# soniareilly/HPCClassMultigridProject

Hardware: NVIDIA B200
Metric: V-cycle ms at N=16384^2 (fine-grid V-cycle incl. convergence check) (lower is better)
Workload: dtype f64

## Files before the change

hpcclassmultigridproject_b200/csrc/solver.cu:

```cuda
#include <cmath>
#include <cstdlib>
#include <cstring>
#include <mutex>
#include <string>
#include <utility>
#include <vector>

#include "comm.cuh"
#include "ops_basic.cuh"
#include "stream_pass.cuh"

namespace mgb200 {

static thread_local std::string g_last_error;
void set_error(const std::string& msg) { g_last_error = msg; }
int fail(int code, const std::string& msg)
{
    g_last_error = msg;
    return code;
}
long& launch_counter()
{
    static thread_local long c = 0;
    return c;
}

Stencil make_stencil(double dt, double nu, double dx)
{
    volatile double r = 0.5 * dt / (dx * dx);
    volatile double four_r = 4.0 * r;
    volatile double four_r_nu = four_r * nu;
    Stencil s;
    s.r = r; s.nu = nu; s.h = dx;
    s.diag = 1.0 - four_r_nu;
    s.diag_rhs = 1.0 + four_r_nu;
    s.inv_diag = 1.0 / s.diag;
    s.hr = r * dx * 0.5;
    s.rnu = r * nu;
    return s;
}

struct Level {
    long n = 0;
    Layout L{0, 0};
    Stencil st{};
    size_t elems = 0;
    double* u[2] = {nullptr, nullptr};
    int cur = 0;
    double *rhs = nullptr, *v1 = nullptr, *v2 = nullptr;
    long own_lo = 0, own_hi = 0;
    long mem_lo = 0, mem_hi = 0;
    bool sharded = false;
    bool present = true;
    long rows_mem() const { return mem_hi - mem_lo + 1; }
};

constexpr long SLAB_HALO = 8;

struct Slab { long own_lo, own_hi, mem_lo, mem_hi; };
static Slab slab_of(long n, int P, int rank)
{
    Slab w;
    const long per = n / P;
    w.own_lo = rank * per;
    w.own_hi = (rank + 1) * per - 1 + (rank == P - 1 ? 1 : 0);
    w.mem_lo = w.own_lo - SLAB_HALO < 0 ? 0 : w.own_lo - SLAB_HALO;
    w.mem_hi = w.own_hi + SLAB_HALO > n ? n : w.own_hi + SLAB_HALO;
    return w;
}
static Slab child_slab_of(long n_fine, int P, int rank)
{
    const Slab f = slab_of(n_fine, P, rank);
    const long nc = n_fine / 2;
    Slab w;
    w.own_lo = (f.own_lo + 1) / 2;
    w.own_hi = f.own_hi / 2;
    w.mem_lo = w.own_lo - SLAB_HALO < 0 ? 0 : w.own_lo - SLAB_HALO;
    w.mem_hi = w.own_hi + SLAB_HALO > nc ? nc : w.own_hi + SLAB_HALO;
    return w;
}

struct LoopState {
    double res0, tol;
    int iter, max_cycle;
    double hist[52];
};

__global__ void k_loop_begin(cudaGraphConditionalHandle h, const double* norm2, LoopState* st, double tol, int max_cycle)
{
    const double r0 = sqrt(norm2[0]);
    st->res0 = r0; st->tol = tol; st->iter = 0; st->max_cycle = max_cycle; st->hist[0] = r0;
    cudaGraphSetConditional(h, (0 < max_cycle && r0 / r0 > tol) ? 1u : 0u);
}

__global__ void k_loop_check(cudaGraphConditionalHandle h, const double* norm2, LoopState* st)
{
    const double r = sqrt(norm2[0]);
    const int it = ++st->iter;
    st->hist[it] = r;
    cudaGraphSetConditional(h, (it < st->max_cycle && r / st->res0 > st->tol) ? 1u : 0u);
}

}

using namespace mgb200;

struct mgb200_solver {
    long N = 0;
    int maxlvl = 0;
    double nu = 0, dt = 0, dx = 0, tol = 0;
    mgb200_options opt{};
    int device = 0;
    std::vector<Level> lv;
    cudaStream_t stream = nullptr;
    double* d_partials = nullptr;
    long partials_cap = 0;
    double* d_norm2 = nullptr;
    double* h_norm2 = nullptr;
    int* d_coarse_iters = nullptr;
    double* d_coarse_lu = nullptr;
    double* d_flat[2] = {nullptr, nullptr};
    cudaGraphExec_t graph_exec = nullptr;
    long graph_kernels = 0;
    cudaGraphExec_t loop_exec = nullptr;
    bool loop_failed = false;
    long loop_kernels = 0;
    LoopState* d_loop = nullptr;
    LoopState* h_loop = nullptr;
    int  build_loop_graph();
    LoopState* h_steps = nullptr;
    int h_steps_cap = 0;
    int  timestep(int nsteps, mgb200_solve_info* infos);
    bool device_loop() const { return opt.use_graph && !loop_failed && (P == 1 || p2p); }
    long launches = 0;
    bool have_fields = false, have_rhs = false;
    bool norm_is_res0 = false;
    bool res0_on_host = false;
    double res0 = 0, res = 0;
    Comm* comm = nullptr;
    int rank = 0, P = 1;
    int last_sharded = -1;
    long shard_min_rows = 256;
    double* d_top[3] = {nullptr, nullptr, nullptr};
    struct PeerLevel { double* u[2] = {nullptr, nullptr}; double* rhs = nullptr; };
    struct PeerRank { std::vector<PeerLevel> lv; int* sync = nullptr; double* red = nullptr; };
    bool p2p = false;
    std::vector<PeerRank> peers;
    int* d_sync = nullptr;
    double* d_red = nullptr;
    int  allreduce_norm();
    int  check_peers();
    std::vector<void*> ipc_mapped;
    int  setup_p2p();
    double* d_flat_scratch() { return d_norm2 + 4; }
    bool tracing = false;
    std::vector<std::pair<std::string, cudaEvent_t>> marks;
    void mark(const std::string& name)
    {
        if (!tracing) return;
        cudaEvent_t e; cudaEventCreate(&e); cudaEventRecord(e, stream);
        marks.emplace_back(name, e);
    }
    void dump_marks()
    {
        if (!tracing || marks.empty()) return;
        cudaStreamSynchronize(stream);
        if (rank == 0) {
            std::string line = "MGB200_TRACE";
            for (size_t k = 1; k < marks.size(); ++k) {
                float ms = 0; cudaEventElapsedTime(&ms, marks[k - 1].second, marks[k].second);
                char buf[96]; snprintf(buf, sizeof buf, " | %s %.3f", marks[k].first.c_str(), ms);
                line += buf;
            }
            float tot = 0; cudaEventElapsedTime(&tot, marks.front().second, marks.back().second);
            fprintf(stderr, "%s | total %.3f ms\n", line.c_str(), tot);
        }
        for (auto& m : marks) cudaEventDestroy(m.second);
        marks.clear();
    }

    ~mgb200_solver() { release(); }
    void release();
    int  init(long n, int maxlvl_, double nu_, double dt_, double dx_, double tol_, const mgb200_options* o);
    int  build_towers();
    int  cycle_body(int l);
    int  smooth(Level& g, int iters);
    int  residual_norm_level0();
    int  record_cycle();
    int  run_cycle_async();
    int  read_norm(double* out);
    int  form_rhs(double* res0_out, bool sync = true);
    int  solve(mgb200_solve_info* info);
    int  get_u_natural(double* dst_dev, long ld);
    int  alloc_levels();
    int  alloc_top();
    void fill_pass_window(StreamPassArgs& a, const Level& g, const Level& c) const;
    bool fused_push = false;
    void fill_pass_push(StreamPassArgs& a, const Level& g, const Level& c, bool coarse_rhs_too) const;
    int  exchange_halo(Level& g, double* a, Level* g2 = nullptr, double* a2 = nullptr);
    int  gather_to_root(Level& c, double* arr);
    int  scatter_from_root(Level& c, double* arr);
    bool runs_level(int l) const { return P == 1 || rank == 0 || lv[l].sharded; }
    long count(long before) { long d = launch_counter() - before; launches += d; return d; }
};

void mgb200_solver::release()
{
    if (graph_exec) { cudaGraphExecDestroy(graph_exec); graph_exec = nullptr; }
    if (loop_exec) { cudaGraphExecDestroy(loop_exec); loop_exec = nullptr; }
    cudaFree(d_loop); d_loop = nullptr;
    if (h_loop) { cudaFreeHost(h_loop); h_loop = nullptr; }
    if (h_steps) { cudaFreeHost(h_steps); h_steps = nullptr; h_steps_cap = 0; }
    if (stream) cudaStreamSynchronize(stream);
    for (void* m : ipc_mapped) cudaIpcCloseMemHandle(m);
    ipc_mapped.clear();
    p2p = false;
    for (auto& g : lv) {
        cudaFree(g.u[0]); cudaFree(g.u[1]); cudaFree(g.rhs); cudaFree(g.v1); cudaFree(g.v2);
    }
    lv.clear();
    cudaFree(d_partials); d_partials = nullptr;
    cudaFree(d_norm2); d_norm2 = nullptr;
    cudaFree(d_coarse_iters); d_coarse_iters = nullptr;
    cudaFree(d_coarse_lu); d_coarse_lu = nullptr;
    cudaFree(d_flat[0]); cudaFree(d_flat[1]); d_flat[0] = d_flat[1] = nullptr;
    for (auto& t : d_top) { cudaFree(t); t = nullptr; }
    cudaFree(d_sync); d_sync = nullptr;
    cudaFree(d_red); d_red = nullptr;
    if (comm) { comm_destroy(comm); comm = nullptr; }
    if (h_norm2) { cudaFreeHost(h_norm2); h_norm2 = nullptr; }
    if (stream) { cudaStreamDestroy(stream); stream = nullptr; }
}

int mgb200_solver::init(long n, int maxlvl_, double nu_, double dt_, double dx_, double tol_, const mgb200_options* o)
{
    if (o) {
        if (o->struct_size != (int)sizeof(mgb200_options)) return fail(MGB200_ERR_INVALID, "mgb200_options.struct_size mismatch");
        opt = *o;
    } else {
        mgb200_default_options(&opt);
    }
    if (n < 4 || (n & (n - 1)) != 0) return fail(MGB200_ERR_INVALID, "n must be a power of two >= 4");
    if (maxlvl_ < 1 || (n >> (maxlvl_ - 1)) < 4) return fail(MGB200_ERR_INVALID, "maxlvl out of range for n");
    if ((n >> (maxlvl_ - 1)) > 64)
        return fail(MGB200_ERR_INVALID, "coarsest level must have n <= 64 (on-device coarse solve); raise maxlvl");
    if (opt.shape < 1 || opt.niter < 0 || opt.max_cycle < 0 || opt.max_cycle > 50)
        return fail(MGB200_ERR_INVALID, "bad options (shape >= 1, niter >= 0, 0 <= max_cycle <= 50)");
    if (opt.coarse_exact != 0 && opt.coarse_exact != 1) return fail(MGB200_ERR_INVALID, "options.coarse_exact: 0 or 1");
    if (opt.restriction != MGB200_RESTRICT_INJECT && opt.restriction != MGB200_RESTRICT_FW &&
        (opt.restriction != MGB200_RESTRICT_FW_UNFUSED || opt.plan != MGB200_PLAN_UNFUSED))
        return fail(MGB200_ERR_INVALID, "options.restriction: 0 (injection), 1 (full weighting, UNFUSED plan only) or 2 (full weighting)");
    if (P > 1 && (opt.plan != MGB200_PLAN_FUSED || opt.correct_towers))
        return fail(MGB200_ERR_INVALID, "the sharded solver supports the fused plan with reference-compatible towers only");
    if (opt.niter == 0) {
        if (P > 1) return fail(MGB200_ERR_INVALID, "niter == 0 is not supported by the sharded solver");
        opt.plan = MGB200_PLAN_UNFUSED;
    }
    if (P > 1) { const char* e = getenv("MGB200_SHARDED_GRAPH"); if (e && atoi(e) == 0) opt.use_graph = 0; }
    if (getenv("MGB200_TRACE")) { tracing = true; opt.use_graph = 0; }
    { const char* e = getenv("MGB200_DEVICE_LOOP"); if (e && atoi(e) == 0) loop_failed = true; }
    int ndev = 0;
    if (cudaGetDeviceCount(&ndev) != cudaSuccess || ndev == 0)
        return fail(MGB200_ERR_NO_DEVICE, "no CUDA device visible; this library has no CPU path");
    if (opt.device >= 0) MGB_CUDA(cudaSetDevice(opt.device));
    MGB_CUDA(cudaGetDevice(&device));
    cudaDeviceProp prop;
    MGB_CUDA(cudaGetDeviceProperties(&prop, device));
    if (prop.major != 10)
        return fail(MGB200_ERR_NO_DEVICE, std::string("device is sm_") + std::to_string(prop.major) + std::to_string(prop.minor) +
                                              ", this library is built for sm_100a only");
    N = n; maxlvl = maxlvl_; nu = nu_; dt = dt_; dx = dx_; tol = tol_;
    MGB_CUDA(cudaStreamCreateWithFlags(&stream, cudaStreamNonBlocking));
    MGB_TRY(ops_basic_init());
    if (opt.plan == MGB200_PLAN_FUSED) MGB_TRY(stream_pass_init());
    MGB_TRY(alloc_levels());
    partials_cap = std::max(residual_partials_count(N), stream_pass_tiles(N, lv[0].own_hi - lv[0].own_lo + 1, -1)) + 8;
    MGB_CUDA(cudaMalloc(&d_partials, partials_cap * sizeof(double)));
    MGB_CUDA(cudaMalloc(&d_norm2, 8 * sizeof(double)));
    MGB_CUDA(cudaMemsetAsync(d_norm2, 0, 8 * sizeof(double), stream));
    MGB_CUDA(cudaMalloc(&d_coarse_iters, sizeof(int)));
    MGB_CUDA(cudaMallocHost(&h_norm2, 8 * sizeof(double)));
    MGB_CUDA(cudaMalloc(&d_loop, sizeof(LoopState)));
    MGB_CUDA(cudaMemsetAsync(d_loop, 0, sizeof(LoopState), stream));
    MGB_CUDA(cudaMallocHost(&h_loop, sizeof(LoopState)));
    MGB_CUDA(cudaStreamSynchronize(stream));
    if (P > 1) MGB_TRY(setup_p2p());
    return MGB200_OK;
}

int mgb200_solver::alloc_levels()
{
    lv.resize(maxlvl);
    last_sharded = -1;
    for (int l = 0; l < maxlvl; ++l) {
        Level& g = lv[l];
        g.n = N >> l;
        g.L = split_layout(g.n);
        g.st = make_stencil(dt, nu, dx * (double)(1L << l));
        g.own_lo = 0; g.own_hi = g.n; g.mem_lo = 0; g.mem_hi = g.n; g.sharded = false; g.present = true;
        if (P > 1) {
            const bool can = l < maxlvl - 1 && (g.n / P) >= shard_min_rows && (g.n / P) >= 2 * SLAB_HALO && last_sharded == l - 1;
            if (can) {
                const Slab w = slab_of(g.n, P, rank);
                g.own_lo = w.own_lo; g.own_hi = w.own_hi; g.mem_lo = w.mem_lo; g.mem_hi = w.mem_hi;
                g.sharded = true;
                last_sharded = l;
            } else if (rank != 0) {
                if (l == last_sharded + 1 && l > 0) {
                    const Slab w = child_slab_of(lv[l - 1].n, P, rank);
                    g.own_lo = w.own_lo; g.own_hi = w.own_hi; g.mem_lo = w.mem_lo; g.mem_hi = w.mem_hi;
                } else {
                    g.present = false;
                }
            }
        }
        if (P > 1 && l == 0 && !g.sharded) return fail(MGB200_ERR_INVALID, "level 0 is too small to be cut over the ranks");
        g.L.row0 = g.mem_lo;
        if (!g.present) continue;
        g.elems = (size_t)g.L.pitch * (size_t)g.rows_mem();
        const size_t bytes = g.elems * sizeof(double);
        MGB_CUDA(cudaMalloc(&g.u[0], bytes));
        MGB_CUDA(cudaMalloc(&g.u[1], bytes));
        MGB_CUDA(cudaMalloc(&g.rhs, bytes));
        MGB_CUDA(cudaMalloc(&g.v1, bytes));
        MGB_CUDA(cudaMalloc(&g.v2, bytes));
        MGB_CUDA(cudaMemsetAsync(g.u[0], 0, bytes, stream));
        MGB_CUDA(cudaMemsetAsync(g.u[1], 0, bytes, stream));
        MGB_CUDA(cudaMemsetAsync(g.rhs, 0, bytes, stream));
        MGB_CUDA(cudaMemsetAsync(g.v1, 0, bytes, stream));
        MGB_CUDA(cudaMemsetAsync(g.v2, 0, bytes, stream));
    }
    return MGB200_OK;
}

int mgb200_solver::alloc_top()
{
    const size_t tb = (size_t)(N / 4 + 2) * (N + 1) * sizeof(double);
    for (auto& t : d_top)
        if (!t) MGB_CUDA(cudaMalloc(&t, tb));
    return MGB200_OK;
}

void mgb200_solver::fill_pass_window(StreamPassArgs& a, const Level& g, const Level& c) const
{
    if (P == 1) return;
    a.own_lo = g.own_lo; a.own_hi = g.own_hi;
    a.row0 = g.mem_lo; a.rows_mem = g.rows_mem();
    a.crow0 = c.mem_lo; a.crows_mem = c.rows_mem();
}

void mgb200_solver::fill_pass_push(StreamPassArgs& a, const Level& g, const Level& c, bool coarse_rhs_too) const
{
    if (!(P > 1 && p2p && fused_push && g.sharded)) return;
    const int l = (int)(&g - lv.data());
    const int twin = a.u_out == g.u[0] ? 0 : 1;
    a.sync = d_sync; a.push_rows = SLAB_HALO;
    a.c_own_lo = c.own_lo; a.c_own_hi = c.own_hi;
    for (int d = 0; d < 2; ++d) {
        const int nb = d == 0 ? rank - 1 : rank + 1;
        if (nb < 0 || nb >= P) continue;
        const Slab w = slab_of(g.n, P, nb);
        double* pu = peers[nb].lv[l].u[twin] - w.mem_lo * g.L.pitch;
        double* pc = nullptr;
        if (coarse_rhs_too && c.sharded) pc = peers[nb].lv[l + 1].rhs - slab_of(c.n, P, nb).mem_lo * c.L.pitch;
        if (d == 0) { a.peer_u_up = pu; a.peer_c_up = pc; a.raise_up = peers[nb].sync + SYNC_PASS_DOWN; }
        else { a.peer_u_dn = pu; a.peer_c_dn = pc; a.raise_dn = peers[nb].sync + SYNC_PASS_UP; }
    }
}

int mgb200_solver::setup_p2p()
{
    p2p = false;
    const char* e = getenv("MGB200_P2P");
    const bool want = !(e && atoi(e) == 0) && P <= 8;
    const int nl = last_sharded + 1;
    const int nh = 3 * (nl + 1) + 2;
    MGB_CUDA(cudaMalloc(&d_sync, SYNC_INTS * sizeof(int)));
    MGB_CUDA(cudaMemsetAsync(d_sync, 0, SYNC_INTS * sizeof(int), stream));
    MGB_CUDA(cudaMalloc(&d_red, RED_DOUBLES * sizeof(double)));
    MGB_CUDA(cudaMemsetAsync(d_red, 0, RED_DOUBLES * sizeof(double), stream));
    std::vector<cudaIpcMemHandle_t> mine(nh), all((size_t)nh * P);
    bool ok = want;
    for (int l = 0; l <= nl && ok; ++l) {
        ok = ok && cudaIpcGetMemHandle(&mine[3 * l + 0], lv[l].u[0]) == cudaSuccess;
        ok = ok && cudaIpcGetMemHandle(&mine[3 * l + 1], lv[l].u[1]) == cudaSuccess;
        ok = ok && cudaIpcGetMemHandle(&mine[3 * l + 2], lv[l].rhs) == cudaSuccess;
    }
    ok = ok && cudaIpcGetMemHandle(&mine[3 * (nl + 1)], d_sync) == cudaSuccess;
    ok = ok && cudaIpcGetMemHandle(&mine[3 * (nl + 1) + 1], d_red) == cudaSuccess;
    cudaGetLastError();
    void *d_send = nullptr, *d_recv = nullptr;
    const size_t hb = (size_t)nh * sizeof(cudaIpcMemHandle_t);
    MGB_CUDA(cudaMalloc(&d_send, hb));
    MGB_CUDA(cudaMalloc(&d_recv, hb * P));
    MGB_CUDA(cudaMemcpyAsync(d_send, mine.data(), hb, cudaMemcpyHostToDevice, stream));
    MGB_TRY(comm_allgather_bytes(comm, d_send, d_recv, hb, stream));
    MGB_CUDA(cudaMemcpyAsync(all.data(), d_recv, hb * P, cudaMemcpyDeviceToHost, stream));
    MGB_CUDA(cudaStreamSynchronize(stream));
    cudaFree(d_send); cudaFree(d_recv);
    peers.assign(P, PeerRank{});
    auto open = [&](int r, int idx) -> void* {
        void* ptr = nullptr;
        if (!ok) return nullptr;
        if (cudaIpcOpenMemHandle(&ptr, all[(size_t)r * nh + idx], cudaIpcMemLazyEnablePeerAccess) != cudaSuccess) {
            cudaGetLastError(); ok = false; return nullptr;
        }
        ipc_mapped.push_back(ptr);
        return ptr;
    };
    for (int r = 0; r < P; ++r) {
        if (r == rank) continue;
        const bool neighbour = r == rank - 1 || r == rank + 1;
        const bool agglo = rank == 0 || r == 0;
        if (!neighbour && !agglo) continue;
        PeerRank& pr = peers[r];
        pr.lv.assign(nl + 1, PeerLevel{});
        if (neighbour)
            for (int l = 0; l < nl; ++l) {
                pr.lv[l].u[0] = (double*)open(r, 3 * l + 0);
                pr.lv[l].u[1] = (double*)open(r, 3 * l + 1);
                pr.lv[l].rhs = (double*)open(r, 3 * l + 2);
            }
        if (rank == 0) { pr.lv[nl].u[0] = (double*)open(r, 3 * nl + 0); pr.lv[nl].u[1] = (double*)open(r, 3 * nl + 1); }
        if (r == 0) pr.lv[nl].rhs = (double*)open(r, 3 * nl + 2);
        pr.sync = (int*)open(r, 3 * (nl + 1));
        if (agglo) pr.red = (double*)open(r, 3 * (nl + 1) + 1);
    }
    double flag = ok ? 1.0 : 0.0;
    MGB_CUDA(cudaMemcpyAsync(d_flat_scratch(), &flag, sizeof(double), cudaMemcpyHostToDevice, stream));
    MGB_TRY(comm_allreduce_sum(comm, d_flat_scratch(), 1, stream));
    MGB_CUDA(cudaMemcpyAsync(&flag, d_flat_scratch(), sizeof(double), cudaMemcpyDeviceToHost, stream));
    MGB_CUDA(cudaStreamSynchronize(stream));
    p2p = flag > P - 0.5;
    { const char* f = getenv("MGB200_FUSED_PUSH"); fused_push = p2p && f && atoi(f) != 0; }
    if (!p2p) {
        for (void* m : ipc_mapped) cudaIpcCloseMemHandle(m);
        ipc_mapped.clear();
        peers.clear();
    }
    if (getenv("MGB200_TRACE") && rank == 0) fprintf(stderr, "MGB200_TRACE halo transport: %s\n", p2p ? "peer memory" : "nccl send/recv");
    return MGB200_OK;
}

int mgb200_solver::check_peers()
{
    if (P == 1 || !p2p || !d_sync) return MGB200_OK;
    int flag = 0;
    MGB_CUDA(cudaMemcpyAsync(&flag, d_sync + SYNC_ABORT, sizeof(int), cudaMemcpyDeviceToHost, stream));
    MGB_CUDA(cudaStreamSynchronize(stream));
    if (flag) return fail(MGB200_ERR_STATE, "a peer rank did not arrive within the spin budget of a device-side wait (it failed or left the collective sequence); results are invalid");
    return MGB200_OK;
}

int mgb200_solver::allreduce_norm()
{
    if (P == 1) return MGB200_OK;
    if (!p2p) return comm_allreduce_sum(comm, d_norm2, 1, stream);
    NormReduce a{};
    a.value = d_norm2; a.red = d_red; a.sync = d_sync; a.rank = rank; a.nranks = P;
    if (rank == 0) for (int r = 1; r < P; ++r) { a.peer_red[r] = peers[r].red; a.peer_sync[r] = peers[r].sync; }
    else { a.peer_red[0] = peers[0].red; a.peer_sync[0] = peers[0].sync; }
    return launch_norm_allreduce(a, stream);
}

int mgb200_solver::exchange_halo(Level& g, double* a, Level* g2, double* a2)
{
    if (P == 1) return MGB200_OK;
    if (p2p) {
        PeerPush pp{};
        pp.sync = d_sync;
        if (rank > 0) {
            pp.raise[pp.nraise++] = peers[rank - 1].sync + SYNC_FROM_DOWN;
            pp.wait_slot[pp.nwait] = SYNC_FROM_UP; pp.wait_count[pp.nwait++] = 1;
        }
        if (rank < P - 1) {
            pp.raise[pp.nraise++] = peers[rank + 1].sync + SYNC_FROM_UP;
            pp.wait_slot[pp.nwait] = SYNC_FROM_DOWN; pp.wait_count[pp.nwait++] = 1;
        }
        Level* lvls[2] = {&g, g2};
        double* arrs[2] = {a, a2};
        for (int k = 0; k < 2; ++k) {
            Level* q = lvls[k];
            if (!q || !q->sharded) continue;
            const int l = (int)(q - lv.data());
            const long cnt = SLAB_HALO * q->L.pitch;
            for (int d = 0; d < 2; ++d) {
                const int nb = d == 0 ? rank - 1 : rank + 1;
                if (nb < 0 || nb >= P) continue;
                const PeerLevel& pl = peers[nb].lv[l];
                double* pbase = arrs[k] == q->u[0] ? pl.u[0] : arrs[k] == q->u[1] ? pl.u[1] : arrs[k] == q->rhs ? pl.rhs : nullptr;
                if (!pbase) return fail(MGB200_ERR_INVALID, "exchange_halo: array is not shared with the neighbours");
                const Slab w = slab_of(q->n, P, nb);
                const long row = d == 0 ? q->own_lo : q->own_hi - SLAB_HALO + 1;
                pp.seg[pp.nseg++] = PeerSeg{arrs[k] + (row - q->mem_lo) * q->L.pitch, pbase + (row - w.mem_lo) * q->L.pitch, cnt};
            }
        }
        return launch_peer_push(pp, stream);
    }
    P2P ops[8];
    int n = 0;
    Level* lvls[2] = {&g, g2};
    double* arrs[2] = {a, a2};
    for (int k = 0; k < 2; ++k) {
        Level* q = lvls[k];
        if (!q || !q->sharded) continue;
        double* base = arrs[k];
        const size_t cnt = (size_t)SLAB_HALO * q->L.pitch;
        auto rowptr = [&](long row) { return base + (row - q->mem_lo) * q->L.pitch; };
        if (rank > 0) {
            ops[n++] = P2P{rank - 1, rowptr(q->own_lo), cnt, true};
            ops[n++] = P2P{rank - 1, rowptr(q->own_lo - SLAB_HALO), cnt, false};
        }
        if (rank < P - 1) {
            ops[n++] = P2P{rank + 1, rowptr(q->own_hi - SLAB_HALO + 1), cnt, true};
            ops[n++] = P2P{rank + 1, rowptr(q->own_hi + 1), cnt, false};
        }
    }
    return comm_p2p(comm, ops, n, stream);
}

int mgb200_solver::gather_to_root(Level& c, double* arr)
{
    if (P == 1) return MGB200_OK;
    const long nf = lv[last_sharded].n;
    if (p2p) {
        PeerPush pp{};
        pp.sync = d_sync;
        if (rank == 0) {
            pp.wait_slot[0] = SYNC_GATHER; pp.wait_count[0] = P - 1; pp.nwait = 1;
        } else {
            if (arr != c.rhs) return fail(MGB200_ERR_INVALID, "gather_to_root: only the coarse rhs is shared with rank 0");
            const int lc = (int)(&c - lv.data());
            const Slab w0 = Slab{0, c.n, 0, c.n};
            pp.seg[0] = PeerSeg{arr + (c.own_lo - c.mem_lo) * c.L.pitch, peers[0].lv[lc].rhs + (c.own_lo - w0.mem_lo) * c.L.pitch,
                                (c.own_hi - c.own_lo + 1) * c.L.pitch};
            pp.nseg = 1;
            pp.raise[0] = peers[0].sync + SYNC_GATHER; pp.nraise = 1;
        }
        return launch_peer_push(pp, stream);
    }
    std::vector<P2P> ops;
    if (rank == 0) {
        for (int r = 1; r < P; ++r) {
            const Slab w = child_slab_of(nf, P, r);
            ops.push_back(P2P{r, arr + (w.own_lo - c.mem_lo) * c.L.pitch, (size_t)(w.own_hi - w.own_lo + 1) * c.L.pitch, false});
        }
    } else {
        ops.push_back(P2P{0, arr + (c.own_lo - c.mem_lo) * c.L.pitch, (size_t)(c.own_hi - c.own_lo + 1) * c.L.pitch, true});
    }
    return comm_p2p(comm, ops.data(), (int)ops.size(), stream);
}

int mgb200_solver::scatter_from_root(Level& c, double* arr)
{
    if (P == 1) return MGB200_OK;
    const long nf = lv[last_sharded].n;
    if (p2p) {
        PeerPush pp{};
        pp.sync = d_sync;
        const int lc = (int)(&c - lv.data());
        const int twin = arr == c.u[0] ? 0 : arr == c.u[1] ? 1 : -1;
        if (twin != 0) return fail(MGB200_ERR_STATE, "scatter_from_root: coarse iterate is not in twin 0");
        if (rank == 0) {
            for (int r = 1; r < P; ++r) {
                const Slab w = child_slab_of(nf, P, r);
                pp.seg[pp.nseg++] = PeerSeg{arr + (w.mem_lo - c.mem_lo) * c.L.pitch, peers[r].lv[lc].u[twin],
                                            (w.mem_hi - w.mem_lo + 1) * c.L.pitch};
                pp.raise[pp.nraise++] = peers[r].sync + SYNC_SCATTER;
            }
        } else {
            pp.wait_slot[0] = SYNC_SCATTER; pp.wait_count[0] = 1; pp.nwait = 1;
        }
        return launch_peer_push(pp, stream);
    }
    std::vector<P2P> ops;
    if (rank == 0) {
        for (int r = 1; r < P; ++r) {
            const Slab w = child_slab_of(nf, P, r);
            ops.push_back(P2P{r, arr + (w.mem_lo - c.mem_lo) * c.L.pitch, (size_t)(w.mem_hi - w.mem_lo + 1) * c.L.pitch, true});
        }
    } else {
        ops.push_back(P2P{0, arr, (size_t)c.rows_mem() * c.L.pitch, false});
    }
    return comm_p2p(comm, ops.data(), (int)ops.size(), stream);
}

int mgb200_solver::build_towers()
{
    if (maxlvl == 1) return MGB200_OK;
    if (opt.correct_towers) {
        for (int l = 1; l < maxlvl; ++l) {
            MGB_TRY(launch_restrict(lv[l].v1, lv[l].L, lv[l - 1].v1, lv[l - 1].L, lv[l - 1].n, stream));
            MGB_TRY(launch_restrict(lv[l].v2, lv[l].L, lv[l - 1].v2, lv[l - 1].L, lv[l - 1].n, stream));
        }
        return MGB200_OK;
    }
    const long h = N / 2;
    const size_t fb = (size_t)(h + 1) * (h + 1) * sizeof(double);
    for (int k = 0; k < 2; ++k)
        if (!d_flat[k]) MGB_CUDA(cudaMalloc(&d_flat[k], fb));
    for (int which = 0; which < 2; ++which) {
        const double* src0 = P == 1 ? (which == 0 ? lv[0].v1 : lv[0].v2) : d_top[1 + which];
        const Layout L0 = P == 1 ? lv[0].L : natural_layout(N + 1);
        int cur = 0;
        for (int l = 1; l < maxlvl; ++l) {
            MGB_CUDA(cudaMemsetAsync(d_flat[cur], 0, fb, stream));
            if (l == 1) MGB_TRY(launch_tower_flat(d_flat[cur], src0, true, L0, N, stream));
            else MGB_TRY(launch_tower_flat(d_flat[cur], d_flat[1 - cur], false, L0, N, stream));
            if (lv[l].present) {
                double* dst = which == 0 ? lv[l].v1 : lv[l].v2;
                MGB_TRY(launch_flat_to_level(dst, lv[l].L, d_flat[cur], lv[l].n, stream, lv[l].mem_lo, lv[l].mem_hi));
            }
            cur = 1 - cur;
        }
    }
    return MGB200_OK;
}

int mgb200_solver::smooth(Level& g, int iters)
{
    for (int it = 0; it < iters; ++it) {
        MGB_TRY(launch_gs_colour(g.u[g.cur], g.rhs, g.v1, g.v2, g.n, g.L, g.st, 0, opt.arith, stream));
        MGB_TRY(launch_gs_colour(g.u[g.cur], g.rhs, g.v1, g.v2, g.n, g.L, g.st, 1, opt.arith, stream));
    }
    return MGB200_OK;
}

int mgb200_solver::cycle_body(int l)
{
    Level& g = lv[l];
    const bool split = P > 1 && g.sharded;
    for (int rep = 0; rep < opt.shape; ++rep) {
        if (l == maxlvl - 1) {
            const bool fresh = (l > 0 && rep == 0);
            if (opt.coarse_exact) MGB_TRY(launch_coarse_lu_solve(g.u[g.cur], g.rhs, g.v1, g.v2, d_coarse_lu, g.n, g.L, g.st, fresh, stream));
            else MGB_TRY(launch_coarse_solve(g.u[g.cur], g.rhs, g.v1, g.v2, g.n, g.L, g.st, opt.arith, fresh,
                                             opt.coarse_maxit, opt.coarse_tol, d_coarse_iters, stream));
            continue;
        }
        Level& c = lv[l + 1];
        if (opt.plan == MGB200_PLAN_UNFUSED) {
            MGB_TRY(smooth(g, opt.niter));
            double* tmp = g.u[1 - g.cur];
            MGB_TRY(launch_residual(tmp, g.u[g.cur], g.rhs, g.v1, g.v2, g.n, g.L, g.st, opt.arith, nullptr, stream));
            if (opt.restriction != MGB200_RESTRICT_INJECT) MGB_TRY(launch_restrict_fw(c.rhs, c.L, tmp, g.L, g.n, true, stream));
            else MGB_TRY(launch_restrict_interior(c.rhs, c.L, tmp, g.L, g.n, stream));
            if (l + 1 != maxlvl - 1)
                MGB_CUDA(cudaMemsetAsync(c.u[c.cur], 0, c.elems * sizeof(double), stream));
            MGB_TRY(cycle_body(l + 1));
            MGB_TRY(launch_prolong(g.u[g.cur], g.L, c.u[c.cur], c.L, c.n, true, stream));
            MGB_TRY(smooth(g, opt.niter));
        } else {
            const bool zero_in = (l > 0 && rep == 0);
            int left = opt.niter;
            bool first = true;
            do {
                const int k = left > 3 ? 3 : left;
                left -= k;
                StreamPassArgs a{};
                a.n = g.n; a.L = g.L; a.st = g.st; a.arith = opt.arith;
                a.u_in = (first && zero_in) ? nullptr : g.u[g.cur];
                a.u_out = g.u[1 - g.cur];
                a.rhs = g.rhs; a.v1 = g.v1; a.v2 = g.v2;
                a.iters = k;
                a.Lc = c.L;
                if (left == 0) { a.post = opt.restriction == MGB200_RESTRICT_FW ? POST_FW : POST_INJECT; a.coarse_rhs = c.rhs; }
                fill_pass_window(a, g, c);
                if (split) fill_pass_push(a, g, c, left == 0);
                MGB_TRY(stream_pass(a, stream));
                g.cur = 1 - g.cur;
                first = false;
                if (split && left > 0 && !a.sync) MGB_TRY(exchange_halo(g, g.u[g.cur]));
            } while (left > 0);
            mark("L" + std::to_string(l) + "dn");
            if (split) {
                const bool pushed = p2p && fused_push;
                if (c.sharded) { if (!pushed) MGB_TRY(exchange_halo(g, g.u[g.cur], &c, c.rhs)); }
                else { if (!pushed) MGB_TRY(exchange_halo(g, g.u[g.cur])); MGB_TRY(gather_to_root(c, c.rhs)); }
            }
            mark("L" + std::to_string(l) + "x");
            if (runs_level(l + 1)) MGB_TRY(cycle_body(l + 1));
            if (split && !c.sharded) { mark("sub"); MGB_TRY(scatter_from_root(c, c.u[c.cur])); mark("scat"); }
            left = opt.niter;
            first = true;
            do {
                const int k = left > 3 ? 3 : left;
                left -= k;
                StreamPassArgs a{};
                a.n = g.n; a.L = g.L; a.st = g.st; a.arith = opt.arith;
                a.u_in = g.u[g.cur];
                a.u_out = g.u[1 - g.cur];
                a.rhs = g.rhs; a.v1 = g.v1; a.v2 = g.v2;
                a.iters = k;
                a.Lc = c.L;
                if (first) a.coarse_u = c.u[c.cur];
                if (left == 0 && l == 0 && rep == opt.shape - 1) { a.post = POST_NORM2; a.partials = d_partials; }
                fill_pass_window(a, g, c);
                if (split) fill_pass_push(a, g, c, false);
                MGB_TRY(stream_pass(a, stream));
                g.cur = 1 - g.cur;
                first = false;
                mark("L" + std::to_string(l) + "up");
                if (split && !a.sync) { MGB_TRY(exchange_halo(g, g.u[g.cur])); mark("L" + std::to_string(l) + "x"); }
            } while (left > 0);
        }
    }
    return MGB200_OK;
}

int mgb200_solver::residual_norm_level0()
{
    Level& g = lv[0];
    MGB_TRY(launch_residual(nullptr, g.u[g.cur], g.rhs, g.v1, g.v2, g.n, g.L, g.st, opt.arith, d_partials, stream));
    MGB_TRY(launch_reduce_partials(d_partials, residual_partials_count(g.n), d_norm2, stream));
    return MGB200_OK;
}

int mgb200_solver::record_cycle()
{
    mark("start");
    MGB_TRY(cycle_body(0));
    if (opt.plan == MGB200_PLAN_FUSED && maxlvl > 1) {
        const int last_k = opt.niter == 0 ? 0 : ((opt.niter - 1) % 3) + 1;
        MGB_TRY(launch_reduce_partials(d_partials, stream_pass_tiles(N, lv[0].own_hi - lv[0].own_lo + 1, last_k), d_norm2, stream));
        MGB_TRY(allreduce_norm());
        mark("norm");
    } else {
        MGB_TRY(residual_norm_level0());
    }
    return MGB200_OK;
}

int mgb200_solver::run_cycle_async()
{
    if (!have_rhs) return fail(MGB200_ERR_STATE, "cycle before form_rhs");
    if (!res0_on_host && norm_is_res0) { MGB_TRY(read_norm(&res0)); res0_on_host = true; }
    norm_is_res0 = false;
    if (!opt.use_graph) {
        const long before = launch_counter();
        MGB_TRY(record_cycle());
        count(before);
        dump_marks();
        return MGB200_OK;
    }
    if (!graph_exec) {
        std::vector<int> cur0;
        for (auto& g : lv) cur0.push_back(g.cur);
        cudaGraph_t graph = nullptr;
        const long before = launch_counter();
        MGB_CUDA(cudaStreamBeginCapture(stream, cudaStreamCaptureModeThreadLocal));
        int rc = record_cycle();
        cudaError_t e = cudaStreamEndCapture(stream, &graph);
        graph_kernels = launch_counter() - before;
        launch_counter() = before;
        if (rc != MGB200_OK) { if (graph) cudaGraphDestroy(graph); return rc; }
        if (e != cudaSuccess) return fail(MGB200_ERR_CUDA, std::string("cudaStreamEndCapture: ") + cudaGetErrorString(e));
        for (size_t l = 0; l < lv.size(); ++l)
            if (lv[l].cur != cur0[l]) { cudaGraphDestroy(graph); return fail(MGB200_ERR_STATE, "cycle does not restore buffer parity"); }
        e = cudaGraphInstantiate(&graph_exec, graph, 0);
        cudaGraphDestroy(graph);
        if (e != cudaSuccess) return fail(MGB200_ERR_CUDA, std::string("cudaGraphInstantiate: ") + cudaGetErrorString(e));
    }
    MGB_CUDA(cudaGraphLaunch(graph_exec, stream));
    launches += graph_kernels;
    return MGB200_OK;
}

int mgb200_solver::build_loop_graph()
{
    std::vector<int> cur0;
    for (auto& g : lv) cur0.push_back(g.cur);
    cudaGraph_t graph = nullptr;
    auto bail = [&](const char* what, cudaError_t e) {
        if (graph) cudaGraphDestroy(graph);
        cudaGetLastError();
        loop_failed = true;
        return fail(MGB200_ERR_CUDA, std::string(what) + ": " + cudaGetErrorString(e));
    };
    cudaError_t e = cudaGraphCreate(&graph, 0);
    if (e != cudaSuccess) return bail("cudaGraphCreate", e);
    cudaGraphConditionalHandle h;
    e = cudaGraphConditionalHandleCreate(&h, graph, 0, 0);
    if (e != cudaSuccess) return bail("cudaGraphConditionalHandleCreate", e);
    cudaKernelNodeParams kp{};
    double tol_ = tol; int maxc = opt.max_cycle;
    void* args[] = {&h, &d_norm2, &d_loop, &tol_, &maxc};
    kp.func = (void*)k_loop_begin; kp.gridDim = dim3(1); kp.blockDim = dim3(1); kp.kernelParams = args;
    cudaGraphNode_t n_begin, n_while;
    e = cudaGraphAddKernelNode(&n_begin, graph, nullptr, 0, &kp);
    if (e != cudaSuccess) return bail("cudaGraphAddKernelNode", e);
    cudaGraphNodeParams cp{};
    cp.type = cudaGraphNodeTypeConditional;
    cp.conditional.handle = h; cp.conditional.type = cudaGraphCondTypeWhile; cp.conditional.size = 1;
    e = cudaGraphAddNode(&n_while, graph, &n_begin, 1, &cp);
    if (e != cudaSuccess) return bail("cudaGraphAddNode(conditional)", e);
    cudaGraph_t body = cp.conditional.phGraph_out[0];
    const long before = launch_counter();
    e = cudaStreamBeginCaptureToGraph(stream, body, nullptr, nullptr, 0, cudaStreamCaptureModeThreadLocal);
    if (e != cudaSuccess) return bail("cudaStreamBeginCaptureToGraph", e);
    int rc = record_cycle();
    if (rc == MGB200_OK) { k_loop_check<<<1, 1, 0, stream>>>(h, d_norm2, d_loop); rc = check_launch("k_loop_check"); }
    cudaGraph_t captured = nullptr;
    e = cudaStreamEndCapture(stream, &captured);
    loop_kernels = launch_counter() - before;
    launch_counter() = before;
    if (rc != MGB200_OK) { cudaGraphDestroy(graph); loop_failed = true; return rc; }
    if (e != cudaSuccess) return bail("cudaStreamEndCapture(loop body)", e);
    for (size_t l = 0; l < lv.size(); ++l)
        if (lv[l].cur != cur0[l]) { cudaGraphDestroy(graph); loop_failed = true; return fail(MGB200_ERR_STATE, "cycle does not restore buffer parity"); }
    e = cudaGraphInstantiate(&loop_exec, graph, 0);
    if (e != cudaSuccess) { loop_exec = nullptr; return bail("cudaGraphInstantiate(loop)", e); }
    cudaGraphDestroy(graph);
    return MGB200_OK;
}

int mgb200_solver::read_norm(double* out)
{
    MGB_CUDA(cudaMemcpyAsync(h_norm2, d_norm2, sizeof(double), cudaMemcpyDeviceToHost, stream));
    MGB_CUDA(cudaStreamSynchronize(stream));
    res = std::sqrt(h_norm2[0]);
    if (out) *out = res;
    return MGB200_OK;
}

int mgb200_solver::form_rhs(double* res0_out, bool sync)
{
    if (!have_fields) return fail(MGB200_ERR_STATE, "form_rhs before set_fields");
    Level& g = lv[0];
    const long before = launch_counter();
    if (P == 1) {
        MGB_TRY(launch_compute_rhs(g.rhs, g.u[g.cur], g.v1, g.v2, g.n, g.L, g.st, opt.arith, d_partials, stream));
        MGB_TRY(launch_reduce_partials(d_partials, compute_rhs_partials_count(g.n, g.n - 1, g.L), d_norm2, stream));
    } else {
        const long ilo = g.own_lo < 1 ? 1 : g.own_lo, ihi = g.own_hi > g.n - 1 ? g.n - 1 : g.own_hi;
        MGB_TRY(launch_compute_rhs(g.rhs, g.u[g.cur], g.v1, g.v2, g.n, g.L, g.st, opt.arith, d_partials, stream, ilo, ihi));
        MGB_TRY(launch_reduce_partials(d_partials, compute_rhs_partials_count(g.n, ihi - ilo + 1, g.L), d_norm2, stream));
        MGB_TRY(allreduce_norm());
        MGB_TRY(exchange_halo(g, g.rhs));
    }
    count(before);
    have_rhs = true;
    norm_is_res0 = true; res0_on_host = false;
    if (!sync) return MGB200_OK;
    MGB_TRY(read_norm(&res0));
    res0_on_host = true;
    if (res0_out) *res0_out = res0;
    return MGB200_OK;
}

namespace mgb200 {
bool report_solve(int cycles, int max_cycle, double res0, double res, double tol)
{
    const bool finite = std::isfinite(res) && std::isfinite(res0);
    const bool ok = finite && (res / res0 <= tol || res0 == 0.0);
    if (ok) return true;
    static const bool quiet = [] { const char* e = getenv("MGB200_QUIET"); return e && atoi(e) != 0; }();
    if (!quiet) {
        if (!finite) fprintf(stderr, "mgb200: residual norm is not finite after %d cycle(s) (res0 = %g, res = %g): the iteration diverged\n", cycles, res0, res);
        else fprintf(stderr, "multigrid did not converge in %d cycles (res/res0 = %.3e > tol = %.3e)\n", max_cycle, res / res0, tol);
    }
    return false;
}
}

int mgb200_solver::solve(mgb200_solve_info* info)
{
    if (!have_rhs) return fail(MGB200_ERR_STATE, "solve before form_rhs");
    if (device_loop() && norm_is_res0 && !loop_exec) {
        if (build_loop_graph() != MGB200_OK) {
            fprintf(stderr, "mgb200: device-side solve loop unavailable (%s); using the host loop\n", mgb200_last_error());
            if (P > 1) return MGB200_ERR_CUDA;
        }
    }
    if (device_loop() && norm_is_res0 && loop_exec) {
        MGB_CUDA(cudaGraphLaunch(loop_exec, stream));
        MGB_CUDA(cudaMemcpyAsync(h_loop, d_loop, sizeof(LoopState), cudaMemcpyDeviceToHost, stream));
        MGB_CUDA(cudaStreamSynchronize(stream));
        norm_is_res0 = false; res0_on_host = true;
        const int it = h_loop->iter;
        launches += 1 + (long)it * loop_kernels;
        res0 = h_loop->res0; res = h_loop->hist[it];
        if (info) {
            std::memset(info, 0, sizeof(*info));
            for (int k = 0; k <= it; ++k) info->hist[k] = h_loop->hist[k];
            info->cycles = it; info->res0 = res0; info->res = res; info->converged = (res / res0 <= tol) ? 1 : 0;
        }
        if (rank == 0) report_solve(it, opt.max_cycle, res0, res, tol);
        return check_peers();
    }
    if (!res0_on_host) {
        if (!norm_is_res0) return fail(MGB200_ERR_STATE, "solve: initial residual norm unknown; call form_rhs first");
        MGB_TRY(read_norm(&res0));
        res0_on_host = true;
    }
    double r0 = res0, r = res0;
    int it = 0;
    if (info) { std::memset(info, 0, sizeof(*info)); info->hist[0] = r0; }
    for (; it < opt.max_cycle && r / r0 > tol; ++it) {
        MGB_TRY(run_cycle_async());
        MGB_TRY(read_norm(&r));
        if (info) info->hist[it + 1] = r;
    }
    if (info) { info->cycles = it; info->res0 = r0; info->res = r; info->converged = (r / r0 <= tol) ? 1 : 0; }
    if (rank == 0) report_solve(it, opt.max_cycle, r0, r, tol);
    return MGB200_OK;
}

int mgb200_solver::timestep(int nsteps, mgb200_solve_info* infos)
{
    if (nsteps <= 0) return MGB200_OK;
    int k0 = 0;
    if (device_loop() && !loop_exec) {
        MGB_TRY(form_rhs(nullptr, false));
        MGB_TRY(solve(infos ? &infos[0] : nullptr));
        k0 = 1;
    }
    if (!(device_loop() && loop_exec)) {
        for (int k = k0; k < nsteps; ++k) {
            MGB_TRY(form_rhs(nullptr, false));
            MGB_TRY(solve(infos ? &infos[k] : nullptr));
        }
        return MGB200_OK;
    }
    const int todo = nsteps - k0;
    if (todo <= 0) return MGB200_OK;
    if (h_steps_cap < todo) {
        if (h_steps) cudaFreeHost(h_steps);
        h_steps = nullptr; h_steps_cap = 0;
        MGB_CUDA(cudaMallocHost(&h_steps, (size_t)todo * sizeof(LoopState)));
        h_steps_cap = todo;
    }
    for (int k = 0; k < todo; ++k) {
        MGB_TRY(form_rhs(nullptr, false));
        MGB_CUDA(cudaGraphLaunch(loop_exec, stream));
        MGB_CUDA(cudaMemcpyAsync(&h_steps[k], d_loop, sizeof(LoopState), cudaMemcpyDeviceToHost, stream));
    }
    MGB_CUDA(cudaStreamSynchronize(stream));
    norm_is_res0 = false; res0_on_host = true;
    for (int k = 0; k < todo; ++k) {
        const LoopState& ls = h_steps[k];
        const int it = ls.iter;
        launches += 1 + (long)it * loop_kernels;
        res0 = ls.res0; res = ls.hist[it];
        if (infos) {
            mgb200_solve_info& info = infos[k0 + k];
            std::memset(&info, 0, sizeof(info));
            for (int c = 0; c <= it; ++c) info.hist[c] = ls.hist[c];
            info.cycles = it; info.res0 = res0; info.res = res; info.converged = (res / res0 <= tol) ? 1 : 0;
        }
        if (rank == 0) report_solve(it, opt.max_cycle, res0, res, tol);
    }
    return check_peers();
}

int mgb200_solver::get_u_natural(double* dst_dev, long ld)
{
    Level& g = lv[0];
    const long before = launch_counter();
    MGB_TRY(launch_convert(dst_dev, natural_layout(ld), g.u[g.cur], g.L, g.n, stream, g.own_lo, g.own_hi));
    count(before);
    return MGB200_OK;
}

extern "C" {

int mgb200_version(void) { return MGB200_VERSION; }
const char* mgb200_last_error(void) { return g_last_error.c_str(); }

void mgb200_default_options(mgb200_options* o)
{
    std::memset(o, 0, sizeof(*o));
    o->struct_size = (int)sizeof(mgb200_options);
    o->shape = 1;
    o->niter = 3;
    o->coarse_maxit = 1000;
    o->coarse_tol = 1e-5;
    o->max_cycle = 50;
    o->arith = MGB200_ARITH_FAST;
    o->plan = MGB200_PLAN_FUSED;
    o->correct_towers = 0;
    o->use_graph = 1;
    o->device = -1;
}

int mgb200_create(mgb200_solver** out, long n, int maxlvl, double nu, double dt, double dx, double tol,
                  const mgb200_options* opt)
{
    if (!out) return fail(MGB200_ERR_INVALID, "out == NULL");
    *out = nullptr;
    mgb200_solver* s = new mgb200_solver();
    int rc = s->init(n, maxlvl, nu, dt, dx, tol, opt);
    if (rc != MGB200_OK) { delete s; return rc; }
    *out = s;
    return MGB200_OK;
}

int mgb200_comm_unique_id(unsigned char id[128]) { return comm_unique_id(id); }

int mgb200_create_sharded(mgb200_solver** out, long n, int maxlvl, double nu, double dt, double dx, double tol,
                          const mgb200_options* opt, int rank, int nranks, const unsigned char id[128], long shard_min_rows)
{
    if (!out) return fail(MGB200_ERR_INVALID, "out == NULL");
    *out = nullptr;
    if (nranks < 1 || (nranks & (nranks - 1)) || rank < 0 || rank >= nranks)
        return fail(MGB200_ERR_INVALID, "create_sharded: nranks must be a power of two, 0 <= rank < nranks");
    mgb200_solver* s = new mgb200_solver();
    s->rank = rank; s->P = nranks;
    if (shard_min_rows > 0) s->shard_min_rows = shard_min_rows;
    int rc = MGB200_OK;
    if (nranks > 1) {
        if (opt && opt->device >= 0) cudaSetDevice(opt->device);
        rc = comm_create(&s->comm, rank, nranks, id);
    }
    if (rc == MGB200_OK) rc = s->init(n, maxlvl, nu, dt, dx, tol, opt);
    if (rc != MGB200_OK) { delete s; return rc; }
    *out = s;
    return MGB200_OK;
}

int mgb200_slab_plan(long n, int maxlvl, int nranks, int rank, long shard_min_rows, int lvl, long out[6])
{
    if (!out || lvl < 0 || lvl >= maxlvl || nranks < 1 || rank < 0 || rank >= nranks) return fail(MGB200_ERR_INVALID, "slab_plan: bad argument");
    if (shard_min_rows <= 0) shard_min_rows = 256;
    int last = -1;
    for (int l = 0; l <= lvl; ++l) {
        const long nl = n >> l;
        long w[6] = {0, 1, 0, nl, 0, nl};
        if (nranks > 1) {
            const bool can = l < maxlvl - 1 && (nl / nranks) >= shard_min_rows && (nl / nranks) >= 2 * SLAB_HALO && last == l - 1;
            if (can) {
                const Slab q = slab_of(nl, nranks, rank);
                w[0] = 1; w[2] = q.own_lo; w[3] = q.own_hi; w[4] = q.mem_lo; w[5] = q.mem_hi;
                last = l;
            } else if (rank != 0) {
                if (l == last + 1 && l > 0) {
                    const Slab q = child_slab_of(n >> (l - 1), nranks, rank);
                    w[2] = q.own_lo; w[3] = q.own_hi; w[4] = q.mem_lo; w[5] = q.mem_hi;
                } else {
                    w[1] = 0;
                }
            }
        }
        if (l == lvl) std::memcpy(out, w, sizeof(w));
    }
    return MGB200_OK;
}

int mgb200_slab(mgb200_solver* s, int lvl, long out[6])
{
    if (!s || !out || lvl < 0 || lvl >= s->maxlvl) return fail(MGB200_ERR_INVALID, "slab: bad argument");
    const Level& g = s->lv[lvl];
    out[0] = g.sharded; out[1] = g.present; out[2] = g.own_lo; out[3] = g.own_hi; out[4] = g.mem_lo; out[5] = g.mem_hi;
    return MGB200_OK;
}

int mgb200_destroy(mgb200_solver* s)
{
    if (!s) return MGB200_OK;
    cudaSetDevice(s->device);
    if (s->stream) cudaStreamSynchronize(s->stream);
    delete s;
    return MGB200_OK;
}

static int after_fields(mgb200_solver* s)
{
    MGB_TRY(s->build_towers());
    if (s->opt.coarse_exact && (s->P == 1 || s->rank == 0)) {
        Level& c = s->lv[s->maxlvl - 1];
        if (!s->d_coarse_lu) MGB_CUDA(cudaMalloc(&s->d_coarse_lu, coarse_lu_bytes(c.n)));
        MGB_TRY(launch_coarse_lu_factor(s->d_coarse_lu, c.v1, c.v2, c.n, c.L, c.st, s->stream));
    }
    if (s->P > 1) {
        MGB_CUDA(cudaStreamSynchronize(s->stream));
        for (auto& t : s->d_top) { cudaFree(t); t = nullptr; }
        cudaFree(s->d_flat[0]); cudaFree(s->d_flat[1]); s->d_flat[0] = s->d_flat[1] = nullptr;
    }
    s->have_fields = true;
    s->have_rhs = false;
    return MGB200_OK;
}

int mgb200_set_fields_device(mgb200_solver* s, const double* u0, const double* v1, const double* v2, long ld)
{
    if (!s || !u0 || !v1 || !v2 || ld < s->N + 1) return fail(MGB200_ERR_INVALID, "set_fields_device: bad argument");
    Level& g = s->lv[0];
    const long before = launch_counter();
    MGB_TRY(launch_convert(g.u[g.cur], g.L, u0, natural_layout(ld), g.n, s->stream, g.mem_lo, g.mem_hi));
    MGB_TRY(launch_convert(g.v1, g.L, v1, natural_layout(ld), g.n, s->stream, g.mem_lo, g.mem_hi));
    MGB_TRY(launch_convert(g.v2, g.L, v2, natural_layout(ld), g.n, s->stream, g.mem_lo, g.mem_hi));
    if (s->P > 1) {
        MGB_TRY(s->alloc_top());
        const long top = s->N / 4 + 1;
        MGB_TRY(launch_convert(s->d_top[1], natural_layout(s->N + 1), v1, natural_layout(ld), s->N, s->stream, 0, top));
        MGB_TRY(launch_convert(s->d_top[2], natural_layout(s->N + 1), v2, natural_layout(ld), s->N, s->stream, 0, top));
    }
    MGB_TRY(after_fields(s));
    s->count(before);
    MGB_CUDA(cudaStreamSynchronize(s->stream));
    return MGB200_OK;
}

int mgb200_set_fields_host(mgb200_solver* s, const double* u0, const double* v1, const double* v2)
{
    if (!s || !u0 || !v1 || !v2) return fail(MGB200_ERR_INVALID, "set_fields_host: bad argument");
    Level& g = s->lv[0];
    const long n = g.n;
    const size_t off = (size_t)g.mem_lo * (n + 1);
    const size_t bytes = (size_t)g.rows_mem() * (n + 1) * sizeof(double);
    const Layout dense = natural_layout(n + 1, g.mem_lo);
    double* stage_a = g.u[1 - g.cur];
    double* stage_b = g.rhs;
    const long before = launch_counter();
    const long top = s->N / 4 + 1;
    auto towers_from_stage = [&](double* stage, double* dtop) -> int {
        const long a = g.own_lo, b = g.own_hi < top ? g.own_hi : top;
        if (a <= b)
            MGB_CUDA(cudaMemcpyAsync(dtop + (size_t)a * (n + 1), stage + (size_t)(a - g.mem_lo) * (n + 1), (size_t)(b - a + 1) * (n + 1) * sizeof(double),
                                     cudaMemcpyDeviceToDevice, s->stream));
        for (int r = 0; r < s->P; ++r) {
            const Slab w = slab_of(g.n, s->P, r);
            const long ra = w.own_lo, rb = w.own_hi < top ? w.own_hi : top;
            if (ra <= rb) MGB_TRY(comm_broadcast(s->comm, dtop + (size_t)ra * (n + 1), (size_t)(rb - ra + 1) * (n + 1), r, s->stream));
        }
        return MGB200_OK;
    };
    if (s->P > 1) MGB_TRY(s->alloc_top());
    MGB_CUDA(cudaMemcpyAsync(stage_a, u0 + off, bytes, cudaMemcpyHostToDevice, s->stream));
    MGB_TRY(launch_convert(g.u[g.cur], g.L, stage_a, dense, n, s->stream, g.mem_lo, g.mem_hi));
    MGB_CUDA(cudaMemcpyAsync(stage_b, v1 + off, bytes, cudaMemcpyHostToDevice, s->stream));
    MGB_TRY(launch_convert(g.v1, g.L, stage_b, dense, n, s->stream, g.mem_lo, g.mem_hi));
    if (s->P > 1) MGB_TRY(towers_from_stage(stage_b, s->d_top[1]));
    MGB_CUDA(cudaMemcpyAsync(stage_a, v2 + off, bytes, cudaMemcpyHostToDevice, s->stream));
    MGB_TRY(launch_convert(g.v2, g.L, stage_a, dense, n, s->stream, g.mem_lo, g.mem_hi));
    if (s->P > 1) MGB_TRY(towers_from_stage(stage_a, s->d_top[2]));
    MGB_CUDA(cudaMemsetAsync(stage_a, 0, g.elems * sizeof(double), s->stream));
    MGB_CUDA(cudaMemsetAsync(stage_b, 0, g.elems * sizeof(double), s->stream));
    MGB_TRY(after_fields(s));
    s->count(before);
    MGB_CUDA(cudaStreamSynchronize(s->stream));
    return MGB200_OK;
}

int mgb200_set_fields_reference_ic(mgb200_solver* s, double vscale)
{
    if (!s) return fail(MGB200_ERR_INVALID, "solver == NULL");
    Level& g = s->lv[0];
    const long before = launch_counter();
    MGB_TRY(launch_initial_conditions(g.u[g.cur], g.v1, g.v2, g.n, g.L, vscale, s->stream, g.mem_lo, g.mem_hi));
    if (s->P > 1) {
        MGB_TRY(s->alloc_top());
        MGB_TRY(launch_initial_conditions(s->d_top[0], s->d_top[1], s->d_top[2], g.n, natural_layout(g.n + 1), vscale, s->stream, 0, s->N / 4 + 1));
    }
    MGB_TRY(after_fields(s));
    s->count(before);
    return MGB200_OK;
}

int mgb200_form_rhs(mgb200_solver* s, double* res0)
{
    if (!s) return fail(MGB200_ERR_INVALID, "solver == NULL");
    return s->form_rhs(res0);
}

int mgb200_cycle(mgb200_solver* s, double* res)
{
    if (!s) return fail(MGB200_ERR_INVALID, "solver == NULL");
    MGB_TRY(s->run_cycle_async());
    return s->read_norm(res);
}

int mgb200_cycle_async(mgb200_solver* s)
{
    if (!s) return fail(MGB200_ERR_INVALID, "solver == NULL");
    return s->run_cycle_async();
}

int mgb200_last_norm(mgb200_solver* s, double* res)
{
    if (!s) return fail(MGB200_ERR_INVALID, "solver == NULL");
    return s->read_norm(res);
}

int mgb200_solve(mgb200_solver* s, mgb200_solve_info* info)
{
    if (!s) return fail(MGB200_ERR_INVALID, "solver == NULL");
    return s->solve(info);
}

int mgb200_timestep(mgb200_solver* s, int nsteps, mgb200_solve_info* infos)
{
    if (!s) return fail(MGB200_ERR_INVALID, "solver == NULL");
    return s->timestep(nsteps, infos);
}

int mgb200_get_u_device(mgb200_solver* s, double* u, long ld)
{
    if (!s || !u || ld < s->N + 1) return fail(MGB200_ERR_INVALID, "get_u_device: bad argument");
    MGB_TRY(s->get_u_natural(u, ld));
    MGB_CUDA(cudaStreamSynchronize(s->stream));
    return MGB200_OK;
}

int mgb200_get_u_host(mgb200_solver* s, double* u)
{
    if (!s || !u) return fail(MGB200_ERR_INVALID, "get_u_host: bad argument");
    Level& g = s->lv[0];
    double* stage = g.u[1 - g.cur];
    const long before = launch_counter();
    MGB_TRY(launch_convert(stage, natural_layout(g.n + 1, g.own_lo), g.u[g.cur], g.L, g.n, s->stream, g.own_lo, g.own_hi));
    s->count(before);
    MGB_CUDA(cudaMemcpyAsync(u + (size_t)g.own_lo * (g.n + 1), stage, (size_t)(g.own_hi - g.own_lo + 1) * (g.n + 1) * sizeof(double),
                             cudaMemcpyDeviceToHost, s->stream));
    MGB_CUDA(cudaStreamSynchronize(s->stream));
    return MGB200_OK;
}

int mgb200_get_level_host(mgb200_solver* s, int lvl, int which, double* out)
{
    if (!s || !out || lvl < 0 || lvl >= s->maxlvl || which < 0 || which > 3) return fail(MGB200_ERR_INVALID, "get_level_host: bad argument");
    Level& g = s->lv[lvl];
    if (!g.present) return MGB200_OK;
    const double* src = which == 0 ? g.u[g.cur] : which == 1 ? g.rhs : which == 2 ? g.v1 : g.v2;
    double* tmp = nullptr;
    const size_t bytes = (size_t)g.rows_mem() * (g.n + 1) * sizeof(double);
    out += (size_t)g.mem_lo * (g.n + 1);
    MGB_CUDA(cudaMalloc(&tmp, bytes));
    int rc = launch_convert(tmp, natural_layout(g.n + 1, g.mem_lo), src, g.L, g.n, s->stream, g.mem_lo, g.mem_hi);
    if (rc == MGB200_OK) {
        cudaError_t e = cudaMemcpyAsync(out, tmp, bytes, cudaMemcpyDeviceToHost, s->stream);
        if (e == cudaSuccess) e = cudaStreamSynchronize(s->stream);
        if (e != cudaSuccess) rc = fail(MGB200_ERR_CUDA, cudaGetErrorString(e));
    }
    cudaFree(tmp);
    return rc;
}

int mgb200_synchronize(mgb200_solver* s)
{
    if (!s) return fail(MGB200_ERR_INVALID, "solver == NULL");
    MGB_CUDA(cudaStreamSynchronize(s->stream));
    return s->check_peers();
}

void* mgb200_stream(mgb200_solver* s) { return s ? (void*)s->stream : nullptr; }
long mgb200_kernel_launches(mgb200_solver* s) { return s ? s->launches : 0; }

double mgb200_cycle_bytes(mgb200_solver* s)
{
    if (!s) return 0.0;
    double total = 0.0;
    for (int l = 0; l < s->maxlvl; ++l) {
        const double m = (double)(s->lv[l].n + 1) * (double)(s->lv[l].n + 1);
        const int reps = 1;
        double per_node;
        if (l == s->maxlvl - 1) {
            per_node = 40.0;
        } else if (s->opt.plan == MGB200_PLAN_UNFUSED) {
            per_node = 2.0 * s->opt.niter * 40.0 + 40.0 + 4.0 + 2.0 + 26.0;
        } else {
            const int chunks = s->opt.niter <= 3 ? 1 : (s->opt.niter + 2) / 3;
            const double down = (l > 0 ? 32.0 : 40.0) + 2.0 + (chunks - 1) * 40.0;
            const double up = 40.0 + 2.0 + (chunks - 1) * 40.0;
            per_node = down + up;
        }
        double mult = 1.0;
        for (int k = 0; k < l; ++k) mult *= s->opt.shape;
        total += per_node * m * mult * reps;
    }
    if (s->opt.plan == MGB200_PLAN_UNFUSED || s->maxlvl == 1) total += 32.0 * (double)(s->N + 1) * (double)(s->N + 1);
    return total;
}

int mgb200_profile_level0(mgb200_solver* s, int reps, double* ms_a, double* bytes_a, double* ms_b, double* bytes_b)
{
    if (!s || reps < 1 || !s->have_rhs) return fail(MGB200_ERR_STATE, "profile_level0: needs a formed rhs");
    if (s->maxlvl < 2) return fail(MGB200_ERR_INVALID, "profile_level0: needs at least two levels");
    Level& g = s->lv[0];
    Level& c = s->lv[1];
    const double m0 = (double)(g.own_hi - g.own_lo + 1) * (double)(g.n + 1);
    cudaEvent_t e0, e1;
    MGB_CUDA(cudaEventCreate(&e0));
    MGB_CUDA(cudaEventCreate(&e1));
    double acc[2] = {0.0, 0.0};
    const long before = launch_counter();
    int rc = MGB200_OK;
    for (int which = 0; which < 2 && rc == MGB200_OK; ++which) {
        for (int r = 0; r < reps && rc == MGB200_OK; ++r) {
            cudaEventRecord(e0, s->stream);
            if (s->opt.plan == MGB200_PLAN_FUSED) {
                StreamPassArgs a{};
                a.n = g.n; a.L = g.L; a.st = g.st; a.arith = s->opt.arith;
                a.u_in = g.u[g.cur]; a.u_out = g.u[1 - g.cur];
                a.rhs = g.rhs; a.v1 = g.v1; a.v2 = g.v2;
                a.iters = s->opt.niter > 3 ? 3 : s->opt.niter;
                a.Lc = c.L;
                if (which == 0) { a.post = s->opt.restriction == MGB200_RESTRICT_FW ? POST_FW : POST_INJECT; a.coarse_rhs = c.rhs; }
                else { a.coarse_u = c.u[c.cur]; a.post = POST_NORM2; a.partials = s->d_partials; }
                s->fill_pass_window(a, g, c);
                rc = stream_pass(a, s->stream);
                g.cur = 1 - g.cur;
            } else if (which == 0) {
                rc = launch_gs_colour(g.u[g.cur], g.rhs, g.v1, g.v2, g.n, g.L, g.st, r & 1, s->opt.arith, s->stream);
            } else {
                rc = launch_residual(g.u[1 - g.cur], g.u[g.cur], g.rhs, g.v1, g.v2, g.n, g.L, g.st, s->opt.arith, nullptr, s->stream);
            }
            cudaEventRecord(e1, s->stream);
            cudaEventSynchronize(e1);
            float ms = 0.f;
            cudaEventElapsedTime(&ms, e0, e1);
            acc[which] += ms;
        }
    }
    s->count(before);
    cudaEventDestroy(e0);
    cudaEventDestroy(e1);
    MGB_TRY(rc);
    if (ms_a) *ms_a = acc[0] / reps;
    if (ms_b) *ms_b = acc[1] / reps;
    const bool fused = s->opt.plan == MGB200_PLAN_FUSED;
    if (bytes_a) *bytes_a = (fused ? 42.0 : 24.0) * m0;
    if (bytes_b) *bytes_b = (fused ? 42.0 : 40.0) * m0;
    return MGB200_OK;
}

namespace {
struct CachedHandle {
    std::mutex mu;
    mgb200_solver* s = nullptr;
    long n = 0; int maxlvl = 0; double nu = 0, dt = 0, dx = 0, tol = 0;
    mgb200_options opt{};
};
CachedHandle g_cached;
}

static int timestepper_common(double* uT, const double* u0, const double* v1, const double* v2, double nu, int maxlvl,
                              int n, double dt, double T, double dx, double tol, int shape, const mgb200_options* opt,
                              mgb200_solve_info* last, bool host)
{
    mgb200_options o;
    if (opt) o = *opt; else mgb200_default_options(&o);
    o.shape = shape;
    std::lock_guard<std::mutex> lock(g_cached.mu);
    const bool reuse = g_cached.s && g_cached.n == n && g_cached.maxlvl == maxlvl && g_cached.nu == nu && g_cached.dt == dt &&
                       g_cached.dx == dx && g_cached.tol == tol && std::memcmp(&g_cached.opt, &o, sizeof(o)) == 0;
    if (!reuse) {
        if (g_cached.s) { mgb200_destroy(g_cached.s); g_cached.s = nullptr; }
        MGB_TRY(mgb200_create(&g_cached.s, n, maxlvl, nu, dt, dx, tol, &o));
        g_cached.n = n; g_cached.maxlvl = maxlvl; g_cached.nu = nu; g_cached.dt = dt; g_cached.dx = dx; g_cached.tol = tol;
        g_cached.opt = o;
    }
    mgb200_solver* s = g_cached.s;
    MGB_CUDA(cudaSetDevice(s->device));
    int rc = host ? mgb200_set_fields_host(s, u0, v1, v2) : mgb200_set_fields_device(s, u0, v1, v2, n + 1);
    const int nsteps = (int)(T / dt);
    mgb200_solve_info info;
    std::memset(&info, 0, sizeof(info));
    if (rc == MGB200_OK && nsteps > 0) {
        std::vector<mgb200_solve_info> infos((size_t)nsteps);
        rc = s->timestep(nsteps, infos.data());
        if (rc == MGB200_OK) info = infos.back();
    }
    if (rc == MGB200_OK) rc = host ? mgb200_get_u_host(s, uT) : mgb200_get_u_device(s, uT, n + 1);
    if (last) *last = info;
    const char* keep = getenv("MGB200_TIMESTEPPER_CACHE");
    if (rc != MGB200_OK || (keep && keep[0] == '0')) { mgb200_destroy(s); g_cached.s = nullptr; }
    return rc;
}

int mgb200_release_cached(void)
{
    std::lock_guard<std::mutex> lock(g_cached.mu);
    if (g_cached.s) { mgb200_destroy(g_cached.s); g_cached.s = nullptr; }
    return MGB200_OK;
}

int mgb200_timestepper_host(double* uT, const double* u0, const double* v1, const double* v2, double nu, int maxlvl,
                            int n, double dt, double T, double dx, double tol, int shape, const mgb200_options* opt,
                            mgb200_solve_info* last)
{
    if (!uT || !u0 || !v1 || !v2) return fail(MGB200_ERR_INVALID, "timestepper: NULL array");
    return timestepper_common(uT, u0, v1, v2, nu, maxlvl, n, dt, T, dx, tol, shape, opt, last, true);
}

int mgb200_timestepper_device(double* uT, const double* u0, const double* v1, const double* v2, double nu, int maxlvl,
                              int n, double dt, double T, double dx, double tol, int shape, const mgb200_options* opt,
                              mgb200_solve_info* last)
{
    if (!uT || !u0 || !v1 || !v2) return fail(MGB200_ERR_INVALID, "timestepper: NULL array");
    return timestepper_common(uT, u0, v1, v2, nu, maxlvl, n, dt, T, dx, tol, shape, opt, last, false);
}

}
```

hpcclassmultigridproject_b200/csrc/stream_pass.cuh:

```cuda
#pragma once
#include "common.cuh"

namespace mgb200 {

enum StreamPost {
    POST_NONE = 0,
    POST_INJECT = 1,
    POST_NORM2 = 2,
    POST_FW = 3
};

struct StreamPassArgs {
    long n;
    Layout L;
    Stencil st;
    const double* u_in;
    double* u_out;
    const double* rhs;
    const double* v1;
    const double* v2;
    int iters;
    const double* coarse_u;
    Layout Lc;
    int post;
    double* coarse_rhs;
    double* partials;
    int arith;
    long own_lo, own_hi;
    long row0, rows_mem;
    long crow0, crows_mem;
    double* peer_u_up; double* peer_u_dn;
    double* peer_c_up; double* peer_c_dn;
    long push_rows;
    long c_own_lo, c_own_hi;
    int* sync;
    int* raise_up; int* raise_dn;
};

long stream_pass_tiles(long n, long nrows, int iters);
int stream_pass_init();
int stream_pass(const StreamPassArgs& a, cudaStream_t s);

}
```

hpcclassmultigridproject_b200/csrc/syst_pass.cu:

```cuda
#include <cuda.h>

#include <algorithm>
#include <cstdlib>
#include <cstring>
#include <map>
#include <mutex>
#include <string>
#include <tuple>

#include "comm.cuh"
#include "syst_pass_body.cuh"

namespace mgb200 {
namespace sy {

__device__ __forceinline__ unsigned smem_u32(const void* p) { return (unsigned)__cvta_generic_to_shared(p); }

SY_FN int sy_lane() { return threadIdx.x & 31; }

SY_FN bool sy_elect()
{
    unsigned pred;
    asm volatile(
        "{\n\t.reg .pred p;\n\t"
        "elect.sync _|p, 0xffffffff;\n\t"
        "selp.u32 %0, 1, 0, p;\n\t}"
        : "=r"(pred));
    return pred != 0;
}

SY_FN void sy_syncwarp() { __syncwarp(); }

SY_FN void sy_full_expect(const Smem& sm, int g, unsigned bytes)
{
    asm volatile("mbarrier.arrive.expect_tx.shared::cta.b64 _, [%0], %1;" ::"r"(sm.base32 + sm.full_off + 8u * g), "r"(bytes) : "memory");
}

SY_FN void sy_tma_load(const Params& p, const Smem& sm, int which, unsigned soff, int x, int z, int g)
{
    asm volatile(
        "cp.async.bulk.tensor.3d.shared::cluster.global.tile.mbarrier::complete_tx::bytes [%0], [%1, {%2, %3, %4}], [%5];" ::"r"(
            sm.base32 + soff),
        "l"(&p.maps[which]), "r"(x), "r"(0), "r"(z), "r"(sm.base32 + sm.full_off + 8u * g)
        : "memory");
}

SY_FN void sy_tma_prefetch(const Params& p, int which, int x, int z)
{
    asm volatile("cp.async.bulk.prefetch.tensor.3d.L2.global.tile [%0, {%1, %2, %3}];" ::"l"(&p.maps[which]), "r"(x), "r"(0), "r"(z)
                 : "memory");
}

__device__ __forceinline__ void mbar_wait(unsigned a, unsigned parity)
{
    unsigned done;
    do {
        asm volatile(
            "{\n\t.reg .pred p;\n\t"
            "mbarrier.try_wait.parity.shared::cta.b64 p, [%1], %2;\n\t"
            "selp.u32 %0, 1, 0, p;\n\t}"
            : "=r"(done)
            : "r"(a), "r"(parity)
            : "memory");
    } while (!done);
}

SY_FN void sy_full_wait(const Smem& sm, int g, unsigned parity) { mbar_wait(sm.base32 + sm.full_off + 8u * g, parity); }

SY_FN void sy_prog_publish(const Smem& sm, int warp, unsigned steps_done)
{
    asm volatile("st.release.cta.shared.u32 [%0], %1;" ::"r"(sm.base32 + sm.pb_off + 4u * (unsigned)warp), "r"(steps_done) : "memory");
}

SY_FN Prog2 sy_prog_peek(const Smem& sm, int stage)
{
    Prog2 v;
    asm volatile("ld.acquire.cta.shared.v2.u32 {%0, %1}, [%2];" : "=r"(v.h0), "=r"(v.h1) : "r"(sm.base32 + sm.pb_off + 8u * (unsigned)stage) : "memory");
    return v;
}

SY_FN void sy_backoff(int ns)
{
    if (ns > 0) __nanosleep((unsigned)ns);
}

SY_FN void sy_wait_neighbour(int* sync, int slot)
{
    const int want = *reinterpret_cast<volatile int*>(sync + SYNC_PASSES_DONE);
    int seen;
    const long long t0 = clock64();
    do {
        asm volatile("ld.acquire.sys.global.s32 %0, [%1];" : "=r"(seen) : "l"(sync + slot) : "memory");
        if (seen - want < 0 && clock64() - t0 > SYNC_SPIN_BUDGET) { sync[SYNC_ABORT] = 1; break; }
    } while (seen - want < 0);
    asm volatile("fence.proxy.async;" ::: "memory");
}

SY_FN void sy_bulk_store(const Smem& sm, double* gdst, unsigned soff, unsigned bytes)
{
    asm volatile("cp.async.bulk.global.shared::cta.bulk_group [%0], [%1], %2;" ::"l"(gdst), "r"(sm.base32 + soff), "r"(bytes) : "memory");
}

SY_FN void sy_store_commit() { asm volatile("cp.async.bulk.commit_group;" ::: "memory"); }
SY_FN void sy_store_wait_read0() { asm volatile("cp.async.bulk.wait_group.read 0;" ::: "memory"); }
SY_FN void sy_store_wait_read1() { asm volatile("cp.async.bulk.wait_group.read 1;" ::: "memory"); }
SY_FN void sy_store_wait_all() { asm volatile("cp.async.bulk.wait_group 0;" ::: "memory"); }
SY_FN void sy_fence_async() { asm volatile("fence.proxy.async.shared::cta;" ::: "memory"); }

SY_FN D2 sy_lds2(const Smem& sm, unsigned off)
{
    D2 v;
    asm volatile("ld.shared.v2.f64 {%0, %1}, [%2];" : "=d"(v.x), "=d"(v.y) : "r"(sm.base32 + off));
    return v;
}
SY_FN double sy_lds1(const Smem& sm, unsigned off)
{
    double v;
    asm volatile("ld.shared.f64 %0, [%1];" : "=d"(v) : "r"(sm.base32 + off));
    return v;
}
SY_FN void sy_sts2(const Smem& sm, unsigned off, D2 v)
{
    asm volatile("st.shared.v2.f64 [%0], {%1, %2};" ::"r"(sm.base32 + off), "d"(v.x), "d"(v.y) : "memory");
}
SY_FN void sy_sts1(const Smem& sm, unsigned off, double v)
{
    asm volatile("st.shared.f64 [%0], %1;" ::"r"(sm.base32 + off), "d"(v) : "memory");
}

SY_FN double sy_side(const Smem& sm, const D2& mid, unsigned off, int dir, bool outer)
{
    const int lane = threadIdx.x & 31;
    double x = dir < 0 ? __shfl_up_sync(0xffffffffu, mid.y, 1) : __shfl_down_sync(0xffffffffu, mid.x, 1);
    if (lane == (dir < 0 ? 0 : 31)) x = outer ? 0.0 : sy_lds1(sm, off);
    return x;
}

template <int ARITH, bool PRE, int POSTK>
__global__ void __launch_bounds__(THREADS, 1) k_syst_pass(const __grid_constant__ Params p)
{
    extern __shared__ __align__(128) unsigned char smem_raw[];
    __shared__ double scratch[32];
    Smem sm;
    carve(sm, smem_raw, p.SWK);
    sm.base32 = smem_u32(smem_raw);
    const Tile tl = make_tile(p, blockIdx.x, POSTK == POST_FW ? 1 : 0);
    const Geo geo = make_geo(p);
    const int warp = __shfl_sync(0xffffffffu, (int)(threadIdx.x >> 5), 0);
    const int lane = threadIdx.x & 31;
    if (threadIdx.x < NGROUP)
        asm volatile("mbarrier.init.shared::cta.b64 [%0], 1;" ::"r"(sm.base32 + sm.full_off + 8u * threadIdx.x) : "memory");
    if (threadIdx.x < NPROG) *reinterpret_cast<volatile unsigned*>(smem_raw + sm.pb_off + 4u * threadIdx.x) = 0u;
    asm volatile("fence.mbarrier_init.release.cluster;" ::: "memory");
    sy_fence_async();
    if (p.sync && threadIdx.x == 0) {
        if (p.raise_up && tl.R0 - 8 < (int)p.own_lo) sy_wait_neighbour(p.sync, SYNC_PASS_UP);
        if (p.raise_dn && tl.R1 + 8 > (int)p.own_hi) sy_wait_neighbour(p.sync, SYNC_PASS_DOWN);
    }
    __syncthreads();
    const double acc = run_warp<ARITH, PRE, POSTK>(p, tl, geo, sm, warp, lane);
    if (p.sync) {
        const bool pushed = (p.raise_up && tl.rb0 < (int)(p.own_lo + 2 * p.push_rows + 2)) || (p.raise_dn && tl.rb1 > (int)(p.own_hi - 2 * p.push_rows - 2));
        if (pushed) __threadfence_system();
        __syncthreads();
        if (threadIdx.x == 0) {
            unsigned* ctas = reinterpret_cast<unsigned*>(p.sync + SYNC_PASS_CTAS);
            if (atomicInc(ctas, gridDim.x - 1) == gridDim.x - 1) {
                __threadfence_system();
                if (p.raise_up) atomicAdd_system(p.raise_up, 1);
                if (p.raise_dn) atomicAdd_system(p.raise_dn, 1);
                p.sync[SYNC_PASSES_DONE] += 1;
            }
        }
    }
    if (POSTK == POST_NORM2) {
        const double tot = block_sum(acc, scratch);
        if (threadIdx.x == 0) p.partials[blockIdx.x] = tot;
    }
}

static int g_sms = 0;

typedef CUresult (*EncodeTiledFn)(CUtensorMap*, CUtensorMapDataType, cuuint32_t, void*, const cuuint64_t*, const cuuint64_t*,
                                  const cuuint32_t*, const cuuint32_t*, CUtensorMapInterleave, CUtensorMapSwizzle,
                                  CUtensorMapL2promotion, CUtensorMapFloatOOBfill);
static EncodeTiledFn g_encode = nullptr;

static int encode_field(TensorMapStorage* out, const double* base, long odd, long pitch, long rows, int box_x, int box_rows)
{
    static_assert(sizeof(CUtensorMap) == sizeof(TensorMapStorage), "CUtensorMap size");
    CUtensorMap m;
    const cuuint64_t dims[3] = {(cuuint64_t)odd, 2, (cuuint64_t)rows};
    const cuuint64_t strides[2] = {(cuuint64_t)odd * 8, (cuuint64_t)pitch * 8};
    const cuuint32_t box[3] = {(cuuint32_t)box_x, 2, (cuuint32_t)box_rows};
    const cuuint32_t estr[3] = {1, 1, 1};
    CUresult r = g_encode(&m, CU_TENSOR_MAP_DATA_TYPE_FLOAT64, 3, const_cast<double*>(base), dims, strides, box, estr,
                          CU_TENSOR_MAP_INTERLEAVE_NONE, CU_TENSOR_MAP_SWIZZLE_NONE, CU_TENSOR_MAP_L2_PROMOTION_L2_256B,
                          CU_TENSOR_MAP_FLOAT_OOB_FILL_NONE);
    if (r != CUDA_SUCCESS) return fail(MGB200_ERR_CUDA, "cuTensorMapEncodeTiled failed with CUresult " + std::to_string((int)r));
    std::memcpy(out, &m, sizeof(m));
    return MGB200_OK;
}

static Plan plan_for(long n, long nrows, int K)
{
    static std::map<std::tuple<long, long, int>, Plan> cache;
    static std::mutex mu;
    std::lock_guard<std::mutex> lock(mu);
    auto key = std::make_tuple(n, nrows, K);
    auto it = cache.find(key);
    if (it == cache.end()) {
        int force = 0;
        if (const char* e = getenv("MGB200_SWK")) force = atoi(e);
        it = cache.emplace(key, make_plan(n, nrows, K, g_sms > 0 ? g_sms : 148, force)).first;
    }
    return it->second;
}

using PassKernel = void (*)(const Params);
template <int ARITH>
static PassKernel pass_kernel_of(bool pre, int post)
{
    if (pre) return post == POST_NORM2 ? k_syst_pass<ARITH, true, POST_NORM2> : post == POST_INJECT ? k_syst_pass<ARITH, true, POST_INJECT>
                                                                                                   : k_syst_pass<ARITH, true, POST_NONE>;
    return post == POST_NORM2 ? k_syst_pass<ARITH, false, POST_NORM2> : post == POST_INJECT ? k_syst_pass<ARITH, false, POST_INJECT>
                                                                                             : k_syst_pass<ARITH, false, POST_NONE>;
}
static PassKernel pass_kernel(int arith, bool pre, int post)
{
    if (post == POST_FW) return arith == MGB200_ARITH_EXACT ? k_syst_pass<MGB200_ARITH_EXACT, false, POST_FW> : k_syst_pass<MGB200_ARITH_FAST, false, POST_FW>;
    return arith == MGB200_ARITH_EXACT ? pass_kernel_of<MGB200_ARITH_EXACT>(pre, post) : pass_kernel_of<MGB200_ARITH_FAST>(pre, post);
}

}

using namespace sy;

int stream_pass_init()
{
    static std::mutex mu;
    static bool done[64] = {};
    int dev = 0;
    MGB_CUDA(cudaGetDevice(&dev));
    std::lock_guard<std::mutex> lock(mu);
    if (dev >= 0 && dev < 64 && done[dev]) return MGB200_OK;
    MGB_CUDA(cudaDeviceGetAttribute(&g_sms, cudaDevAttrMultiProcessorCount, dev));
    for (int arith = 0; arith < 2; ++arith)
        for (int pre = 0; pre < 2; ++pre)
            for (int post = 0; post < 3; ++post)
                MGB_CUDA(cudaFuncSetAttribute(pass_kernel(arith, pre != 0, post), cudaFuncAttributeMaxDynamicSharedMemorySize, (int)SMEM_BYTES));
    for (int arith = 0; arith < 2; ++arith)
        MGB_CUDA(cudaFuncSetAttribute(pass_kernel(arith, false, POST_FW), cudaFuncAttributeMaxDynamicSharedMemorySize, (int)SMEM_BYTES));
    if (!g_encode) {
        void* fn = nullptr;
        cudaDriverEntryPointQueryResult qres;
        MGB_CUDA(cudaGetDriverEntryPoint("cuTensorMapEncodeTiled", &fn, cudaEnableDefault, &qres));
        if (!fn || qres != cudaDriverEntryPointSuccess) return fail(MGB200_ERR_CUDA, "cuTensorMapEncodeTiled not available from the driver");
        g_encode = (EncodeTiledFn)fn;
    }
    if (dev >= 0 && dev < 64) done[dev] = true;
    return MGB200_OK;
}

long stream_pass_tiles(long n, long nrows, int iters)
{
    if (iters >= 1) {
        const Plan pl = plan_for(n, nrows, iters > KMAX ? KMAX : iters);
        return (long)pl.nstrips * pl.nbands;
    }
    long m = 0;
    for (int K = 1; K <= KMAX; ++K) {
        const Plan pl = plan_for(n, nrows, K);
        m = std::max(m, (long)pl.nstrips * pl.nbands);
    }
    return m;
}

static int build_params(const StreamPassArgs& a, Params& p, unsigned& grid_out, size_t& smem_out)
{
    if (a.iters < 1 || a.iters > KMAX) return fail(MGB200_ERR_INVALID, "stream_pass: iters must be 1..3");
    if (a.n < 8 || (a.n & 3)) return fail(MGB200_ERR_INVALID, "stream_pass: n must be a multiple of 4, >= 8");
    if (!a.L.split() || a.u_out == a.u_in) return fail(MGB200_ERR_INVALID, "stream_pass: needs the split layout and u_out != u_in");
    MGB_TRY(stream_pass_init());
    const bool whole = a.rows_mem == 0;
    const long own_lo = whole ? 0 : a.own_lo, own_hi = whole ? a.n : a.own_hi;
    const Plan pl = plan_for(a.n, own_hi - own_lo + 1, a.iters);
    p = Params{};
    p.n = a.n; p.nhalf = a.n / 2;
    p.own_lo = own_lo; p.own_hi = own_hi;
    p.row0 = whole ? 0 : a.row0; p.rows_mem = whole ? a.n + 1 : a.rows_mem;
    p.mem_lo = p.row0; p.mem_hi = p.row0 + p.rows_mem - 1;
    p.crow0 = whole ? 0 : a.crow0; p.crows_mem = whole ? a.n / 2 + 1 : a.crows_mem;
    p.pitch = a.L.pitch; p.odd = a.L.odd;
    p.cpitch = a.Lc.pitch; p.codd = a.Lc.odd;
    p.RBAND = pl.RBAND; p.WK = pl.WK; p.SWK = pl.SWK; p.nstrips = pl.nstrips; p.nbands = pl.nbands;
    p.K = a.iters;
    p.pre = a.coarse_u ? 1 : 0;
    p.post = a.post;
    p.u_is_zero = a.u_in ? 0 : 1;
    p.CW = pl.SWK / 2 + 8;
    { const char* e = getenv("MGB200_SY_BACKOFF"); p.backoff_ns = e ? atoi(e) : 0; }
    p.st = a.st;
    p.u_in = a.u_in; p.rhs = a.rhs; p.v1 = a.v1; p.v2 = a.v2; p.cu = a.coarse_u;
    MGB_TRY(encode_field(&p.maps[FIELD_U], a.u_in ? a.u_in : a.rhs, a.L.odd, a.L.pitch, p.rows_mem, pl.SWK, GROUP));
    MGB_TRY(encode_field(&p.maps[FIELD_F], a.rhs, a.L.odd, a.L.pitch, p.rows_mem, pl.SWK, GROUP));
    MGB_TRY(encode_field(&p.maps[FIELD_V1], a.v1, a.L.odd, a.L.pitch, p.rows_mem, pl.SWK, GROUP));
    MGB_TRY(encode_field(&p.maps[FIELD_V2], a.v2, a.L.odd, a.L.pitch, p.rows_mem, pl.SWK, GROUP));
    if (a.coarse_u) MGB_TRY(encode_field(&p.maps[FIELD_C], a.coarse_u, a.Lc.odd, a.Lc.pitch, p.crows_mem, p.CW, CROWS));
    p.u_out = a.u_out; p.crhs = a.coarse_rhs; p.partials = a.partials;
    p.peer_u_up = a.peer_u_up; p.peer_u_dn = a.peer_u_dn; p.peer_c_up = a.peer_c_up; p.peer_c_dn = a.peer_c_dn;
    p.push_rows = a.push_rows; p.c_own_lo = a.c_own_lo; p.c_own_hi = a.c_own_hi;
    p.sync = a.sync; p.raise_up = a.raise_up; p.raise_dn = a.raise_dn;
    if (p.post == POST_INJECT && !p.crhs) return fail(MGB200_ERR_INVALID, "stream_pass: POST_INJECT without coarse_rhs");
    if (p.post == POST_FW && (!p.crhs || p.pre)) return fail(MGB200_ERR_INVALID, "stream_pass: POST_FW needs coarse_rhs and no prolongation");
    if (p.post == POST_NORM2 && !p.partials) return fail(MGB200_ERR_INVALID, "stream_pass: POST_NORM2 without partials");
    grid_out = (unsigned)(pl.nstrips * pl.nbands);
    smem_out = smem_bytes(pl.SWK);
    return MGB200_OK;
}

int stream_pass(const StreamPassArgs& a, cudaStream_t s)
{
    struct Entry { Params p; unsigned grid; size_t smem; };
    static std::map<std::string, Entry> cache;
    static std::mutex mu;
    Entry e;
    {
        std::lock_guard<std::mutex> lock(mu);
        StreamPassArgs key;
        std::memset(&key, 0, sizeof(key));
        key.n = a.n; key.L = a.L; key.st = a.st; key.u_in = a.u_in; key.u_out = a.u_out; key.rhs = a.rhs; key.v1 = a.v1; key.v2 = a.v2;
        key.iters = a.iters; key.coarse_u = a.coarse_u; key.Lc = a.Lc; key.post = a.post; key.coarse_rhs = a.coarse_rhs;
        key.partials = a.partials; key.arith = a.arith; key.own_lo = a.own_lo; key.own_hi = a.own_hi; key.row0 = a.row0;
        key.rows_mem = a.rows_mem; key.crow0 = a.crow0; key.crows_mem = a.crows_mem;
        key.peer_u_up = a.peer_u_up; key.peer_u_dn = a.peer_u_dn; key.peer_c_up = a.peer_c_up; key.peer_c_dn = a.peer_c_dn;
        key.push_rows = a.push_rows; key.c_own_lo = a.c_own_lo; key.c_own_hi = a.c_own_hi; key.sync = a.sync;
        key.raise_up = a.raise_up; key.raise_dn = a.raise_dn;
        std::string k(reinterpret_cast<const char*>(&key), sizeof(key));
        auto it = cache.find(k);
        if (it == cache.end()) {
            Entry fresh;
            MGB_TRY(build_params(a, fresh.p, fresh.grid, fresh.smem));
            if (cache.size() > 4096) cache.clear();
            it = cache.emplace(std::move(k), fresh).first;
        }
        e = it->second;
    }
    pass_kernel(a.arith, e.p.pre != 0, e.p.post)<<<e.grid, THREADS, e.smem, s>>>(e.p);
    return check_launch("k_syst_pass");
}

}
```

hpcclassmultigridproject_b200/csrc/syst_pass_body.cuh:

```cuda
#pragma once
#include "common.cuh"
#include "stream_pass.cuh"

#ifndef SY_FN
#define SY_FN __device__ __forceinline__
#endif

namespace mgb200 {
namespace sy {

constexpr int SWK_MAX = 128;
constexpr int HK = 4;
constexpr int GROUP = 4;
constexpr int RING = 24;
constexpr int NGROUP = RING / GROUP;
constexpr int CROWS = 3;
constexpr int KMAX = 3;
constexpr int NSTW = 2;
constexpr int NPAIR = 2 * KMAX + 2;
constexpr int NSTAGE = NPAIR * NSTW;
constexpr int WARPS = NSTAGE + 2;
constexpr int THREADS = WARPS * 32;
constexpr int PRODUCER_WARP = NSTAGE;
constexpr int STORE_WARP = NSTAGE + 1;
constexpr int NPROG = NSTAGE + 2;
constexpr int FW_ROWS = 8;
struct alignas(64) TensorMapStorage { unsigned long long q[16]; };

struct Params {
    TensorMapStorage maps[5];
    long n, nhalf;
    long pitch, odd;
    long cpitch, codd;
    long RBAND;
    long own_lo, own_hi;
    long mem_lo, mem_hi;
    long row0, crow0;
    long rows_mem, crows_mem;
    int WK, SWK;
    int nstrips, nbands;
    int K;
    int pre;
    int post;
    int u_is_zero;
    int CW;
    int backoff_ns;
    Stencil st;
    const double* u_in;
    const double* rhs;
    const double* v1;
    const double* v2;
    const double* cu;
    double* u_out;
    double* crhs;
    double* partials;
    double* peer_u_up; double* peer_u_dn; double* peer_c_up; double* peer_c_dn;
    long push_rows, c_own_lo, c_own_hi;
    int* sync; int* raise_up; int* raise_dn;
};

struct Tile {
    int R0, R1;
    int rb0, rb1;
    int k0;
    int kb;
};

struct Smem {
    unsigned char* raw;
    unsigned base32;
    unsigned full_off;
    unsigned pb_off;
};

enum Field { FIELD_U = 0, FIELD_F = 1, FIELD_V1 = 2, FIELD_V2 = 3, FIELD_C = 4 };

constexpr size_t smem_bytes(int swk)
{
    return (size_t)4 * RING * 2 * swk * 8 + (size_t)NGROUP * CROWS * 2 * (swk / 2 + 8) * 8 + NGROUP * 8 + NPROG * 4 + 128;
}
constexpr size_t SMEM_BYTES = smem_bytes(SWK_MAX);

struct alignas(16) D2 { double x, y; };

SY_FN void carve(Smem& sm, unsigned char* base, int swk)
{
    sm.raw = base; sm.base32 = 0;
    sm.full_off = (unsigned)(4 * RING * 2 * swk * 8 + NGROUP * CROWS * 2 * (swk / 2 + 8) * 8);
    sm.pb_off = sm.full_off + NGROUP * 8;
}

SY_FN Tile make_tile(const Params& p, long tile, int extra = 0)
{
    Tile tl;
    const long strip = tile % p.nstrips, band = tile / p.nstrips;
    const long HR = 2 * p.K + 1 + extra;
    long rb0 = p.own_lo + band * p.RBAND, rb1 = rb0 + p.RBAND - 1;
    if (rb1 > p.own_hi) rb1 = p.own_hi;
    long R0 = rb0 - HR, R1 = rb1 + HR;
    if (R0 < p.mem_lo) R0 = p.mem_lo;
    if (R1 > p.mem_hi) R1 = p.mem_hi;
    tl.kb = (int)(strip * p.WK);
    tl.k0 = tl.kb - HK;
    tl.rb0 = (int)rb0; tl.rb1 = (int)rb1; tl.R0 = (int)R0; tl.R1 = (int)R1;
    return tl;
}

SY_FN int  sy_lane();
SY_FN bool sy_elect();
SY_FN void sy_syncwarp();
SY_FN void sy_full_expect(const Smem& sm, int g, unsigned bytes);
SY_FN void sy_tma_load(const Params& p, const Smem& sm, int which, unsigned soff, int x, int z, int g);
SY_FN void sy_tma_prefetch(const Params& p, int which, int x, int z);
SY_FN void sy_full_wait(const Smem& sm, int g, unsigned parity);
struct Prog2 { unsigned h0, h1; };
SY_FN void sy_prog_publish(const Smem& sm, int warp, unsigned steps_done);
SY_FN Prog2 sy_prog_peek(const Smem& sm, int stage);
SY_FN void sy_backoff(int ns);
SY_FN void sy_wait_neighbour(int* sync, int slot);
SY_FN void sy_bulk_store(const Smem& sm, double* gdst, unsigned soff, unsigned bytes);
SY_FN void sy_store_commit();
SY_FN void sy_store_wait_read0();
SY_FN void sy_store_wait_read1();
SY_FN void sy_store_wait_all();
SY_FN void sy_fence_async();
SY_FN D2 sy_lds2(const Smem& sm, unsigned off);
SY_FN double sy_lds1(const Smem& sm, unsigned off);
SY_FN void sy_sts2(const Smem& sm, unsigned off, D2 v);
SY_FN void sy_sts1(const Smem& sm, unsigned off, double v);
SY_FN double sy_side(const Smem& sm, const D2& mid, unsigned off, int dir, bool outer);

struct Geo {
    unsigned swkb;
    unsigned rowb;
    unsigned ringb;
    unsigned cwb;
    unsigned cgrpb;
    int nh;
    int backoff_ns;
};
SY_FN Geo make_geo(const Params& p)
{
    Geo g;
    g.swkb = (unsigned)p.SWK * 8u; g.rowb = 2u * g.swkb; g.ringb = (unsigned)RING * g.rowb;
    g.cwb = (unsigned)p.CW * 8u; g.cgrpb = (unsigned)CROWS * 2u * g.cwb;
    g.nh = p.SWK > 64 ? 2 : 1;
    g.backoff_ns = p.backoff_ns;
    return g;
}

SY_FN unsigned ring_adv(unsigned a, const Geo& g, unsigned lim)
{
    a += g.rowb;
    return a >= lim ? a - g.ringb : a;
}

SY_FN int num_groups(const Tile& tl) { return (tl.R1 - tl.R0) / GROUP + 1; }

constexpr int PAIR_PRE = 2 * KMAX, PAIR_EPI = 2 * KMAX + 1, PAIR_STORE = NPAIR;

SY_FN int off_stage(const Params& p, int s) { return 1 + 2 * s + (p.pre ? 1 : 0); }
SY_FN int off_epi(const Params& p) { return off_stage(p, 2 * p.K - 1) + 2; }
SY_FN int last_step(const Params& p, const Tile& tl, int xr = 0) { return tl.rb1 + xr + (p.post != POST_NONE ? off_epi(p) : off_stage(p, 2 * p.K - 1)); }

struct Stage {
    int pair;
    int up;
    int h;
    int s;
    int kk;
    int off;
    int row;
    int lo, hi;
    unsigned a_prev, a_cur, a_next;
    unsigned lim;
    unsigned okp0, okp1;
    bool outer_l, outer_r;
    bool live;
    D2 c_up, c_mid;
    unsigned rmask0, rmask1;
    int elo, ehi;
    double acc;
    unsigned cmask0, cmask1;
};

struct FwSums { D2 e, o; };

SY_FN Stage init_role(const Params& p, const Tile& tl, const Geo& geo, int pair, int up, int s, int off, int h, int lane)
{
    Stage st;
    st.pair = pair; st.up = up; st.s = s; st.h = h; st.off = off;
    int kk = 64 * h + 2 * lane;
    if (kk > p.SWK - 2) kk = p.SWK - 2;
    const bool live = 64 * h + 2 * lane < p.SWK;
    st.kk = kk;
    st.row = tl.R0 - off;
    st.lo = tl.R0 + 1; st.hi = tl.R1 - 1;
    st.c_up = D2{0.0, 0.0}; st.c_mid = D2{0.0, 0.0};
    st.acc = 0.0;
    st.elo = tl.rb0 < 1 ? 1 : tl.rb0; st.ehi = tl.rb1 > p.n - 1 ? (int)p.n - 1 : tl.rb1;
    st.okp0 = st.okp1 = st.rmask0 = st.rmask1 = st.cmask0 = st.cmask1 = 0;
    for (int e = 0; e < 2 && live; ++e) {
        const int k = kk + e;
        const long kg = (long)tl.k0 + k;
        const bool owned = k >= HK && k < HK + p.WK;
        const bool int0 = kg >= 1 && kg <= p.nhalf - 1;
        const bool int1 = kg >= 0 && kg <= p.nhalf - 1;
        if (int0 && k >= 1) st.okp0 |= 1u << e;
        if (int1 && k <= p.SWK - 2) st.okp1 |= 1u << e;
        if (int0 && owned) st.rmask0 |= 1u << e;
        if (int1 && owned) st.rmask1 |= 1u << e;
        if (int0) st.cmask0 |= 1u << e;
        if (int1) st.cmask1 |= 1u << e;
    }
    st.live = live;
    st.outer_l = kk == 0;
    st.outer_r = kk + 2 >= p.SWK;
    const int slot = ((RING - off) % RING + RING) % RING;
    st.lim = geo.ringb + (unsigned)kk * 8u;
    st.a_cur = (unsigned)slot * geo.rowb + (unsigned)kk * 8u;
    st.a_next = ring_adv(st.a_cur, geo, st.lim);
    st.a_prev = (slot == 0 ? (unsigned)(RING - 1) : (unsigned)(slot - 1)) * geo.rowb + (unsigned)kk * 8u;
    return st;
}

SY_FN void advance_row(const Geo& geo, Stage& st)
{
    st.row += 1;
    st.a_prev = st.a_cur; st.a_cur = st.a_next; st.a_next = ring_adv(st.a_next, geo, st.lim);
}

SY_FN void prog_wait(const Smem& sm, int pair, unsigned need0, unsigned need1, Prog2 pv, int backoff_ns = 0)
{
    while (pv.h0 < need0 || pv.h1 < need1) { sy_backoff(backoff_ns); pv = sy_prog_peek(sm, pair); }
}

SY_FN void wait_inputs(const Tile& tl, const Geo& geo, const Smem& sm, const Stage& st, int k, Prog2 seen)
{
    if (st.up < 0) {
        const int t = tl.R0 + k;
        if ((k & (GROUP - 1)) == 0 && t <= tl.R1) {
            const int g = k / GROUP;
            sy_full_wait(sm, g % NGROUP, (unsigned)(g / NGROUP) & 1u);
        }
    } else {
        prog_wait(sm, st.up, (unsigned)k, geo.nh == 2 ? (unsigned)k : 0u, seen, geo.backoff_ns);
    }
}

SY_FN void publish(const Smem& sm, const Stage& st, int k)
{
    sy_syncwarp();
    if (sy_elect()) sy_prog_publish(sm, st.pair * NSTW + st.h, (unsigned)k + 1u);
}

SY_FN void pre_step(const Params& p, const Tile& tl, const Geo& geo, const Smem& sm, Stage& st, const int k)
{
    const int t = st.row;
    wait_inputs(tl, geo, sm, st, k, Prog2{0u, 0u});
    if (t >= tl.R0 && t <= tl.R1 && t >= 1 && t <= (int)p.n - 1) {
        const int PAR = (t + 1) & 1;
        const unsigned a = st.a_cur + (PAR ? geo.swkb : 0u);
        const int g = k / GROUP, G0 = tl.R0 + g * GROUP;
        const int crow = (t >> 1) - (G0 >> 1);
        const unsigned c0 = 4u * geo.ringb + (unsigned)(g % NGROUP) * geo.cgrpb + (unsigned)crow * 2u * geo.cwb + (unsigned)(st.kk >> 1) * 8u;
        D2 u{0.0, 0.0};
#ifdef SY_HOST_MODEL
        if (st.live)
#endif
        u = sy_lds2(sm, a);
        const double a0 = sy_lds1(sm, c0), a1 = sy_lds1(sm, c0 + geo.cwb);
        D2 e;
        if (PAR) {
            const double a2 = sy_lds1(sm, c0 + 8u);
            e.x = __dmul_rn(__dadd_rn(a0, a1), 0.5); e.y = __dmul_rn(__dadd_rn(a1, a2), 0.5);
        } else {
            const unsigned c1 = c0 + 2u * geo.cwb;
            const double b0 = sy_lds1(sm, c1), b1 = sy_lds1(sm, c1 + geo.cwb);
            e.x = __dmul_rn(__dadd_rn(a0, b0), 0.5); e.y = __dmul_rn(__dadd_rn(a1, b1), 0.5);
        }
        const unsigned cm = PAR ? st.cmask1 : st.cmask0;
        u.x = __dadd_rn(u.x, e.x); u.y = __dadd_rn(u.y, e.y);
        if (cm == 3u) sy_sts2(sm, a, u);
        else {
            if (cm & 1u) sy_sts1(sm, a, u.x);
            if (cm & 2u) sy_sts1(sm, a + 8u, u.y);
        }
    }
    publish(sm, st, k);
    advance_row(geo, st);
}

SY_FN void pre_loop(const Params& p, const Tile& tl, const Geo& geo, const Smem& sm, Stage& st)
{
    const int klast = last_step(p, tl) - tl.R0;
    for (int k = 0; k <= klast; ++k) pre_step(p, tl, geo, sm, st, k);
}

SY_FN void store_coarse(const Params& p, const Stage& st, long kg, long cr, double r0, double r1)
{
    double* crow = p.crhs + (cr - p.crow0) * p.cpitch + (kg >> 1);
    if (st.rmask0 & 1u) crow[0] = r0;
    if (st.rmask0 & 2u) crow[p.codd] = r1;
    if (p.peer_c_up && cr < p.c_own_lo + p.push_rows) {
        double* q = p.peer_c_up + cr * p.cpitch + (kg >> 1);
        if (st.rmask0 & 1u) q[0] = r0;
        if (st.rmask0 & 2u) q[p.codd] = r1;
    }
    if (p.peer_c_dn && cr > p.c_own_hi - p.push_rows) {
        double* q = p.peer_c_dn + cr * p.cpitch + (kg >> 1);
        if (st.rmask0 & 1u) q[0] = r0;
        if (st.rmask0 & 2u) q[p.codd] = r1;
    }
}

SY_FN unsigned fw_off(const Tile& tl, const Geo& geo, const Stage& st, int row)
{
    return 4u * geo.ringb + (unsigned)((row - tl.R0) & (FW_ROWS - 1)) * geo.rowb + (unsigned)st.kk * 8u;
}

SY_FN double fw_row(double a, double b, double c, double w)
{
    return __dmul_rn(__dadd_rn(__dadd_rn(__dmul_rn(w, a), __dmul_rn(2.0 * w, b)), __dmul_rn(w, c)), 0.0625);
}

SY_FN void fw_restrict_row(const Params& p, const Tile& tl, const Geo& geo, const Smem& sm, const Stage& st, FwSums& fw,
                           const int k, const int q, const bool live)
{
    prog_wait(sm, PAIR_EPI, (unsigned)k, geo.nh == 2 ? (unsigned)k : 0u, sy_prog_peek(sm, PAIR_EPI), geo.backoff_ns);
    const unsigned b = fw_off(tl, geo, st, q);
    D2 e{0.0, 0.0}, o{0.0, 0.0};
    if (live) { e = sy_lds2(sm, b); o = sy_lds2(sm, b + geo.swkb); }
    const double ol = sy_side(sm, o, b + geo.swkb - 8u, -1, st.outer_l);
    const double w = (q & 1) ? 1.0 : 2.0;
    const D2 h{fw_row(ol, e.x, o.x, w), fw_row(o.x, e.y, o.y, w)};
    if ((q & 1) == 0) { fw.e = h; return; }
    if (q - 1 >= st.elo && q - 1 <= st.ehi)
        store_coarse(p, st, (long)tl.k0 + st.kk, (long)(q >> 1), __dadd_rn(__dadd_rn(fw.o.x, fw.e.x), h.x),
                     __dadd_rn(__dadd_rn(fw.o.y, fw.e.y), h.y));
    fw.o = h;
}

template <int ARITH, bool LAST, bool NORM1, bool RESID, int EPI, bool FULL>
SY_FN void stage_step(const Params& p, const Tile& tl, const Geo& geo, const Smem& sm, Stage& st, const int k, const int PAR,
                      const bool CHECKED, FwSums* fw)
{
    const unsigned po = PAR ? geo.swkb : 0u, oo = PAR ? 0u : geo.swkb;
    const unsigned c = st.a_cur + po;
    const int row = st.row;
    const bool own_ok = !CHECKED || (row >= tl.R0 && row <= tl.R1);
    const bool dn_ok = !CHECKED || (row + 1 >= tl.R0 && row + 1 <= tl.R1);
#ifdef SY_HOST_MODEL
    const bool live = st.live;
#else
    const bool live = true;
#endif
    Prog2 seen{0u, 0u};
    if (st.up >= 0) seen = sy_prog_peek(sm, st.up);
    Prog2 seen_epi{0u, 0u};
    if (EPI == POST_FW && !RESID) seen_epi = sy_prog_peek(sm, PAIR_EPI);
    const bool work = !RESID || EPI == POST_NORM2 || EPI == POST_FW || PAR == 0;
    D2 f{0.0, 0.0}, w1{0.0, 0.0}, w2{0.0, 0.0}, own{0.0, 0.0};
    double x = 0.0;
    const D2 up = st.c_up, m = st.c_mid;
    if (work && own_ok && live) {
        f = sy_lds2(sm, c + geo.ringb); w1 = sy_lds2(sm, c + 2u * geo.ringb); w2 = sy_lds2(sm, c + 3u * geo.ringb);
        if (RESID) own = sy_lds2(sm, c);
    }
    if (work && own_ok) x = sy_side(sm, m, st.a_cur + oo + (PAR ? 16u : 0u) - (PAR ? 0u : 8u), PAR ? 1 : -1, PAR ? st.outer_r : st.outer_l);
    const double n0 = PAR ? m.x : x, n1 = PAR ? m.y : m.x, n2 = PAR ? x : m.y;
    const Coef4 c0 = Arith<ARITH>::coef(w1.x, w2.x, p.st);
    const Coef4 c1 = Arith<ARITH>::coef(w1.y, w2.y, p.st);
    double h0 = 0.0, h1 = 0.0;
    if (!RESID) { h0 = Arith<ARITH>::gs_head(f.x, up.x, n0, c0); h1 = Arith<ARITH>::gs_head(f.y, up.y, n1, c1); }
    wait_inputs(tl, geo, sm, st, k, seen);
    D2 dn{0.0, 0.0};
    if (dn_ok && live) dn = sy_lds2(sm, st.a_next + po);
    const unsigned rm = PAR ? st.rmask1 : st.rmask0;
    if (!RESID) {
        const double o0 = Arith<ARITH>::gs_tail(h0, dn.x, n1, c0.d, c0.b, p.st);
        const double o1 = Arith<ARITH>::gs_tail(h1, dn.y, n2, c1.d, c1.b, p.st);
        const bool act = FULL || (row >= st.lo && row <= st.hi);
        const unsigned okb = FULL ? 3u : act ? (PAR ? st.okp1 : st.okp0) : 0u;
        if (okb == 3u) sy_sts2(sm, c, D2{o0, o1});
        else {
            if (okb & 1u) sy_sts1(sm, c, o0);
            if (okb & 2u) sy_sts1(sm, c + 8u, o1);
        }
        if (EPI == POST_FW) {
            const int need = k + 5 - FW_ROWS;
            if (need > 0) prog_wait(sm, PAIR_EPI, (unsigned)need, geo.nh == 2 ? (unsigned)need : 0u, seen_epi, geo.backoff_ns);
            const double r0 = Arith<ARITH>::residual(f.x, o0, up.x, n0, dn.x, n1, c0, p.st);
            const double r1 = Arith<ARITH>::residual(f.y, o1, up.y, n1, dn.y, n2, c1, p.st);
            if (live) sy_sts2(sm, fw_off(tl, geo, st, row) + po, D2{r0, r1});
        }
        publish(sm, st, k);
        if (NORM1 && row >= st.elo && row <= st.ehi) {
            const double r0 = Arith<ARITH>::residual(f.x, o0, up.x, n0, dn.x, n1, c0, p.st);
            const double r1 = Arith<ARITH>::residual(f.y, o1, up.y, n1, dn.y, n2, c1, p.st);
            if (rm & 1u) st.acc += r0 * r0;
            if (rm & 2u) st.acc += r1 * r1;
        }
    } else if (EPI == POST_FW) {
        if (own_ok && live) {
            const double r0 = Arith<ARITH>::residual(f.x, own.x, up.x, n0, dn.x, n1, c0, p.st);
            const double r1 = Arith<ARITH>::residual(f.y, own.y, up.y, n1, dn.y, n2, c1, p.st);
            sy_sts2(sm, fw_off(tl, geo, st, row) + po, D2{r0, r1});
        }
        publish(sm, st, k);
        fw_restrict_row(p, tl, geo, sm, st, *fw, k, row - 1, live);
    } else {
        publish(sm, st, k);
        if (work && row >= st.elo && row <= st.ehi && (EPI == POST_NORM2 || (row & 1) == 0)) {
            const double r0 = Arith<ARITH>::residual(f.x, own.x, up.x, n0, dn.x, n1, c0, p.st);
            const double r1 = Arith<ARITH>::residual(f.y, own.y, up.y, n1, dn.y, n2, c1, p.st);
            if (EPI == POST_INJECT) {
                store_coarse(p, st, (long)tl.k0 + st.kk, row >> 1, r0, r1);
            } else {
                if (rm & 1u) st.acc += r0 * r0;
                if (rm & 2u) st.acc += r1 * r1;
            }
        }
    }
    st.c_up = m; st.c_mid = dn;
    advance_row(geo, st);
}

template <int ARITH, bool LAST, bool NORM1, bool RESID, int EPI, int XR = 0>
SY_FN void stage_loop(const Params& p, const Tile& tl, const Geo& geo, const Smem& sm, Stage& st)
{
    const int klast = last_step(p, tl, XR) - tl.R0;
    FwSums fw{D2{0.0, 0.0}, D2{0.0, 0.0}};
    int par = (st.s + st.row) & 1;
    int k = 0;
    const int kchk = st.off + 1;
    int kmain = tl.R1 - tl.R0 + st.off - 1;
    if (kmain > klast) kmain = klast;
    const bool full = !RESID && tl.k0 >= 1 && (long)tl.k0 + p.SWK <= p.nhalf && (p.SWK & 63) == 0;
    for (; k <= klast && (k < kchk || par != 0); ++k, par ^= 1)
        stage_step<ARITH, LAST, NORM1, RESID, EPI, false>(p, tl, geo, sm, st, k, par, true, &fw);
    if (full) {
        for (; k + 1 <= kmain; k += 2) {
            stage_step<ARITH, LAST, NORM1, RESID, EPI, true>(p, tl, geo, sm, st, k, 0, false, &fw);
            stage_step<ARITH, LAST, NORM1, RESID, EPI, true>(p, tl, geo, sm, st, k + 1, 1, false, &fw);
        }
    } else {
        for (; k + 1 <= kmain; k += 2) {
            stage_step<ARITH, LAST, NORM1, RESID, EPI, false>(p, tl, geo, sm, st, k, 0, false, &fw);
            stage_step<ARITH, LAST, NORM1, RESID, EPI, false>(p, tl, geo, sm, st, k + 1, 1, false, &fw);
        }
    }
    for (; k <= klast; ++k, par ^= 1)
        stage_step<ARITH, LAST, NORM1, RESID, EPI, false>(p, tl, geo, sm, st, k, par, true, &fw);
}

SY_FN void issue_group_loads(const Params& p, const Tile& tl, const Geo& geo, const Smem& sm, int g)
{
    if (!sy_elect()) return;
    const int gs = g % NGROUP;
    const int z = tl.R0 + GROUP * g - (int)p.row0;
    const unsigned fine = (unsigned)GROUP * geo.rowb;
    sy_full_expect(sm, gs, 4u * fine + (p.pre ? geo.cgrpb : 0u));
    const unsigned so = (unsigned)gs * fine;
    sy_tma_load(p, sm, FIELD_U, so, tl.k0, p.u_is_zero ? (int)p.rows_mem + 64 : z, gs);
    sy_tma_load(p, sm, FIELD_F, so + geo.ringb, tl.k0, z, gs);
    sy_tma_load(p, sm, FIELD_V1, so + 2u * geo.ringb, tl.k0, z, gs);
    sy_tma_load(p, sm, FIELD_V2, so + 3u * geo.ringb, tl.k0, z, gs);
    if (p.pre)
        sy_tma_load(p, sm, FIELD_C, 4u * geo.ringb + (unsigned)gs * geo.cgrpb, tl.k0 / 2, ((z + (int)p.row0) >> 1) - (int)p.crow0, gs);
    const int zp = z + 2 * GROUP;
    if (g + 2 >= NGROUP && zp + (int)p.row0 <= tl.R1) {
        if (!p.u_is_zero) sy_tma_prefetch(p, FIELD_U, tl.k0, zp);
        sy_tma_prefetch(p, FIELD_F, tl.k0, zp);
        sy_tma_prefetch(p, FIELD_V1, tl.k0, zp);
        sy_tma_prefetch(p, FIELD_V2, tl.k0, zp);
    }
}

template <int XR = 0>
SY_FN void store_loop(const Params& p, const Tile& tl, const Geo& geo, const Smem& sm)
{
    const int klast = last_step(p, tl, XR) - tl.R0;
    const int pair_s = 2 * p.K - 1, off_s = off_stage(p, pair_s);
    long eE = (long)tl.kb + p.WK, eO = eE;
    if (eE > p.nhalf + 1) eE = p.nhalf + 1;
    if (eO > p.nhalf) eO = p.nhalf;
    const unsigned nE8 = (unsigned)(((eE - tl.kb + 1) & ~1L) * 8);
    const unsigned nO8 = (unsigned)((eO - tl.kb) * 8);
    int rs = tl.R0 - off_s;
    const long pitch = p.pitch;
    double* gstE = p.u_out + ((long)rs - p.row0) * pitch + tl.kb;
    double* gstO = gstE + p.odd;
    unsigned a = (unsigned)((((rs - tl.R0) % RING) + RING) % RING) * geo.rowb + (unsigned)HK * 8u;
    const unsigned awrap = geo.ringb + (unsigned)HK * 8u;
    const unsigned need_h1 = geo.nh == 2 ? 1u : 0u;
    const bool push = p.peer_u_up != nullptr || p.peer_u_dn != nullptr;
    Prog2 seen_s{0u, 0u};
    unsigned groups = 0;
    for (int k = 0; k <= klast; ++k, ++rs) {
        const bool store = rs >= tl.rb0 && rs <= tl.rb1;
        const bool close = rs >= tl.R0 && ((rs - tl.R0) & (GROUP - 1)) == GROUP - 1;
        if ((store || close) && (seen_s.h0 < (unsigned)k + 1u || seen_s.h1 < need_h1 * ((unsigned)k + 1u))) {
            seen_s = sy_prog_peek(sm, pair_s);
            while (seen_s.h0 < (unsigned)k + 1u || seen_s.h1 < need_h1 * ((unsigned)k + 1u)) { sy_backoff(geo.backoff_ns); seen_s = sy_prog_peek(sm, pair_s); }
        }
        if (close) ++groups;
        if ((store || close) && sy_elect()) {
            if (store) {
                sy_fence_async();
                if (nE8) sy_bulk_store(sm, gstE, a, nE8);
                if (nO8) sy_bulk_store(sm, gstO, a + geo.swkb, nO8);
                if (push) {
                    if (p.peer_u_up && rs < p.own_lo + p.push_rows) {
                        double* q = p.peer_u_up + (long)rs * pitch + tl.kb;
                        if (nE8) sy_bulk_store(sm, q, a, nE8);
                        if (nO8) sy_bulk_store(sm, q + p.odd, a + geo.swkb, nO8);
                    }
                    if (p.peer_u_dn && rs > p.own_hi - p.push_rows) {
                        double* q = p.peer_u_dn + (long)rs * pitch + tl.kb;
                        if (nE8) sy_bulk_store(sm, q, a, nE8);
                        if (nO8) sy_bulk_store(sm, q + p.odd, a + geo.swkb, nO8);
                    }
                }
            }
            if (close) {
                sy_store_commit();
                sy_store_wait_read0();
                sy_prog_publish(sm, 2 * PAIR_STORE, groups);
            }
        }
        gstE += pitch; gstO += pitch;
        a += geo.rowb;
        if (a >= awrap) a -= geo.ringb;
    }
    if (sy_elect()) { sy_store_commit(); sy_store_wait_all(); sy_prog_publish(sm, 2 * PAIR_STORE, groups + 64u); }
}

template <int XR = 0>
SY_FN void producer_loop(const Params& p, const Tile& tl, const Geo& geo, const Smem& sm)
{
    const int ng = num_groups(tl);
    int gnext = 0;
    for (; gnext < ng && gnext < NGROUP; ++gnext) issue_group_loads(p, tl, geo, sm, gnext);
    const int klast = last_step(p, tl, XR) - tl.R0;
    const int pair_s = 2 * p.K - 1, off_s = off_stage(p, pair_s);
    const bool epi = p.post != POST_NONE;
    const int pair_l = epi ? PAIR_EPI : pair_s, off_l = epi ? off_epi(p) : off_s;
    const unsigned need_h1 = geo.nh == 2 ? 1u : 0u;
    int rl = tl.R0 - off_l;
    for (int k = 0; k <= klast && gnext < ng; ++k, ++rl) {
        if (rl < tl.R0 + GROUP * gnext - RING + GROUP - 1) continue;
        prog_wait(sm, pair_l, (unsigned)k + 1u, need_h1 * ((unsigned)k + 1u), sy_prog_peek(sm, pair_l));
        prog_wait(sm, PAIR_STORE, (unsigned)(gnext - NGROUP + 1), 0u, sy_prog_peek(sm, PAIR_STORE));
        if (sy_elect()) sy_fence_async();
        issue_group_loads(p, tl, geo, sm, gnext);
        ++gnext;
    }
}

template <int ARITH, bool PRE, int POSTK>
SY_FN double run_warp(const Params& p, const Tile& tl, const Geo& geo, const Smem& sm, int warp, int lane)
{
    constexpr int XR = POSTK == POST_FW ? 2 : 0;
    if (warp == PRODUCER_WARP) {
#ifdef SY_HOST_MODEL
        if (lane != 0) return 0.0;
#endif
        producer_loop<XR>(p, tl, geo, sm);
        return 0.0;
    }
    if (warp == STORE_WARP) {
#ifdef SY_HOST_MODEL
        if (lane != 0) return 0.0;
#endif
        store_loop<XR>(p, tl, geo, sm);
        return 0.0;
    }
    const int pair = warp / NSTW, h = warp % NSTW;
    if (h >= geo.nh) return 0.0;
    const int last = 2 * p.K - 1;
    if (pair == PAIR_PRE) {
        if (!PRE) return 0.0;
        Stage st = init_role(p, tl, geo, PAIR_PRE, -1, 1, 0, h, lane);
        pre_loop(p, tl, geo, sm, st);
        return 0.0;
    }
    if (pair == PAIR_EPI) {
        if (POSTK == POST_NONE) return 0.0;
        Stage st = init_role(p, tl, geo, PAIR_EPI, last, 2 * p.K, off_epi(p), h, lane);
        stage_loop<ARITH, false, false, true, POSTK, XR>(p, tl, geo, sm, st);
        return st.acc;
    }
    if (pair > last) return 0.0;
    Stage st = init_role(p, tl, geo, pair, pair == 0 ? (PRE ? PAIR_PRE : -1) : pair - 1, pair, off_stage(p, pair), h, lane);
    if (pair == last && POSTK == POST_NORM2) stage_loop<ARITH, true, true, false, POST_NONE>(p, tl, geo, sm, st);
    else if (pair == last && POSTK == POST_FW) stage_loop<ARITH, true, false, false, POST_FW, XR>(p, tl, geo, sm, st);
    else stage_loop<ARITH, false, false, false, POST_NONE, XR>(p, tl, geo, sm, st);
    return st.acc;
}

struct Plan { int WK, SWK, nstrips, nbands; long RBAND; };

inline Plan make_plan(long n, long nrows, int K, int sms, int force_swk = 0)
{
    const long npairs = n / 2 + 1;
    Plan best{};
    double best_cost = 1e300;
    for (int SWK = 32; SWK <= SWK_MAX; SWK += 16) {
        if (force_swk && SWK != force_swk) continue;
        const int WK = SWK - 2 * HK;
        const int nstrips = (int)((npairs + WK - 1) / WK);
        for (int nb = 1; nb <= 4096; nb = nb < 16 ? nb + 1 : nb * 2) {
            const long RB = (nrows + nb - 1) / nb;
            if (nb > 1 && RB < 8) break;
            const int nbands = (int)((nrows + RB - 1) / RB);
            const long tiles = (long)nstrips * nbands;
            const long waves = (tiles + sms - 1) / sms;
            const double steps = (double)RB + 2.0 * (2 * K + 1) + 4.0 * K + 2.0 * GROUP;
            const double per_step = 96.0 + SWK;
            const double cost = (double)waves * steps * per_step;
            if (cost < best_cost) { best_cost = cost; best = Plan{WK, SWK, nstrips, nbands, RB}; }
        }
    }
    return best;
}

}
}
```

Measured before the change: 6.619.

## Fold right-hand-side formation and initial residual norm into first fine-grid smoothing pass

Adds a FOLD variant of the streaming smoother kernel in which the pre-stage warps compute the time-step right-hand side from u and the coefficient fields in shared memory. That stage writes it back through the store warp and accumulates the initial residual norm, so the separate form_rhs kernel and the F-field load are dropped for the first pass. The solve loop is split into a head part (folded pass plus reduction) and a rest part, with a new CUDA graph using if/while conditional nodes and a matching host fallback. This removes one full fine-grid read/write sweep per timestep. In exchange it adds kernel template variants and more complex graph construction and buffer-parity handling.

```diff
diff --git a/hpcclassmultigridproject_b200/csrc/solver.cu b/hpcclassmultigridproject_b200/csrc/solver.cu
--- a/hpcclassmultigridproject_b200/csrc/solver.cu
+++ b/hpcclassmultigridproject_b200/csrc/solver.cu
@@ -128,6 +128,14 @@
     LoopState* d_loop = nullptr;
     LoopState* h_loop = nullptr;
     int  build_loop_graph();
+    bool fold_enabled = true;
+    enum { CYCLE_ALL, CYCLE_HEAD, CYCLE_REST } cycle_part = CYCLE_ALL;
+    cudaGraphExec_t fold_exec = nullptr;
+    long fold_head_kernels = 0, fold_rest_kernels = 0;
+    bool folds() const { return fold_enabled && opt.plan == MGB200_PLAN_FUSED && maxlvl > 1 && P == 1; }
+    int  record_part(int part);
+    int  build_fold_graph();
+    int  fold_step_host(mgb200_solve_info* info);
     LoopState* h_steps = nullptr;
     int h_steps_cap = 0;
     int  timestep(int nsteps, mgb200_solve_info* infos);
@@ -208,6 +216,7 @@
 {
     if (graph_exec) { cudaGraphExecDestroy(graph_exec); graph_exec = nullptr; }
     if (loop_exec) { cudaGraphExecDestroy(loop_exec); loop_exec = nullptr; }
+    if (fold_exec) { cudaGraphExecDestroy(fold_exec); fold_exec = nullptr; }
     cudaFree(d_loop); d_loop = nullptr;
     if (h_loop) { cudaFreeHost(h_loop); h_loop = nullptr; }
     if (h_steps) { cudaFreeHost(h_steps); h_steps = nullptr; h_steps_cap = 0; }
@@ -259,6 +268,7 @@
     if (P > 1) { const char* e = getenv("MGB200_SHARDED_GRAPH"); if (e && atoi(e) == 0) opt.use_graph = 0; }
     if (getenv("MGB200_TRACE")) { tracing = true; opt.use_graph = 0; }
     { const char* e = getenv("MGB200_DEVICE_LOOP"); if (e && atoi(e) == 0) loop_failed = true; }
+    { const char* e = getenv("MGB200_FOLD_RHS"); if (e && atoi(e) == 0) fold_enabled = false; }
     int ndev = 0;
     if (cudaGetDeviceCount(&ndev) != cudaSuccess || ndev == 0)
         return fail(MGB200_ERR_NO_DEVICE, "no CUDA device visible; this library has no CPU path");
@@ -657,6 +667,8 @@
             do {
                 const int k = left > 3 ? 3 : left;
                 left -= k;
+                const bool head = l == 0 && rep == 0 && first && cycle_part != CYCLE_ALL;
+                if (head && cycle_part == CYCLE_REST) { first = false; continue; }
                 StreamPassArgs a{};
                 a.n = g.n; a.L = g.L; a.st = g.st; a.arith = opt.arith;
                 a.u_in = (first && zero_in) ? nullptr : g.u[g.cur];
@@ -665,11 +677,13 @@
                 a.iters = k;
                 a.Lc = c.L;
                 if (left == 0) { a.post = opt.restriction == MGB200_RESTRICT_FW ? POST_FW : POST_INJECT; a.coarse_rhs = c.rhs; }
+                if (head) { a.fold_rhs = g.rhs; a.partials = d_partials; }
                 fill_pass_window(a, g, c);
                 if (split) fill_pass_push(a, g, c, left == 0);
                 MGB_TRY(stream_pass(a, stream));
                 g.cur = 1 - g.cur;
                 first = false;
+                if (head) return launch_reduce_partials(d_partials, stream_pass_tiles(N, g.own_hi - g.own_lo + 1, k), d_norm2, stream);
                 if (split && left > 0 && !a.sync) MGB_TRY(exchange_halo(g, g.u[g.cur]));
             } while (left > 0);
             mark("L" + std::to_string(l) + "dn");
@@ -814,6 +828,121 @@
     return MGB200_OK;
 }
 
+int mgb200_solver::record_part(int part)
+{
+    cycle_part = part == CYCLE_HEAD ? CYCLE_HEAD : CYCLE_REST;
+    const int rc = part == CYCLE_HEAD ? cycle_body(0) : record_cycle();
+    cycle_part = CYCLE_ALL;
+    return rc;
+}
+
+int mgb200_solver::build_fold_graph()
+{
+    std::vector<int> cur0;
+    for (auto& g : lv) cur0.push_back(g.cur);
+    cudaGraph_t graph = nullptr, part = nullptr;
+    auto bail = [&](const char* what, cudaError_t e) {
+        if (graph) cudaGraphDestroy(graph);
+        if (part) cudaGraphDestroy(part);
+        for (size_t l = 0; l < lv.size(); ++l) lv[l].cur = cur0[l];
+        cudaGetLastError();
+        loop_failed = true;
+        return fail(MGB200_ERR_CUDA, std::string(what) + ": " + cudaGetErrorString(e));
+    };
+    auto failed = [&](int rc) {
+        if (graph) cudaGraphDestroy(graph);
+        for (size_t l = 0; l < lv.size(); ++l) lv[l].cur = cur0[l];
+        loop_failed = true;
+        return rc;
+    };
+    cudaError_t e = cudaGraphCreate(&graph, 0);
+    if (e != cudaSuccess) return bail("cudaGraphCreate", e);
+    cudaGraphConditionalHandle h_if, h_while;
+    e = cudaGraphConditionalHandleCreate(&h_if, graph, 0, 0);
+    if (e == cudaSuccess) e = cudaGraphConditionalHandleCreate(&h_while, graph, 0, cudaGraphCondAssignDefault);
+    if (e != cudaSuccess) return bail("cudaGraphConditionalHandleCreate", e);
+    long before = launch_counter();
+    e = cudaStreamBeginCapture(stream, cudaStreamCaptureModeThreadLocal);
+    if (e != cudaSuccess) return bail("cudaStreamBeginCapture(head)", e);
+    int rc = record_part(CYCLE_HEAD);
+    e = cudaStreamEndCapture(stream, &part);
+    fold_head_kernels = launch_counter() - before + 1;
+    launch_counter() = before;
+    if (rc != MGB200_OK) { if (part) cudaGraphDestroy(part); return failed(rc); }
+    if (e != cudaSuccess) return bail("cudaStreamEndCapture(head)", e);
+    cudaGraphNode_t n_head, n_begin, n_if, n_while;
+    e = cudaGraphAddChildGraphNode(&n_head, graph, nullptr, 0, part);
+    cudaGraphDestroy(part); part = nullptr;
+    if (e != cudaSuccess) return bail("cudaGraphAddChildGraphNode", e);
+    cudaKernelNodeParams kp{};
+    double tol_ = tol; int maxc = opt.max_cycle;
+    void* args[] = {&h_if, &d_norm2, &d_loop, &tol_, &maxc};
+    kp.func = (void*)k_loop_begin; kp.gridDim = dim3(1); kp.blockDim = dim3(1); kp.kernelParams = args;
+    e = cudaGraphAddKernelNode(&n_begin, graph, &n_head, 1, &kp);
+    if (e != cudaSuccess) return bail("cudaGraphAddKernelNode", e);
+    cudaGraphNodeParams cp{};
+    cp.type = cudaGraphNodeTypeConditional;
+    cp.conditional.handle = h_if; cp.conditional.type = cudaGraphCondTypeIf; cp.conditional.size = 1;
+    e = cudaGraphAddNode(&n_if, graph, &n_begin, 1, &cp);
+    if (e != cudaSuccess) return bail("cudaGraphAddNode(if)", e);
+    cudaGraph_t body_if = cp.conditional.phGraph_out[0];
+    cudaGraphNodeParams cw{};
+    cw.type = cudaGraphNodeTypeConditional;
+    cw.conditional.handle = h_while; cw.conditional.type = cudaGraphCondTypeWhile; cw.conditional.size = 1;
+    e = cudaGraphAddNode(&n_while, graph, &n_if, 1, &cw);
+    if (e != cudaSuccess) return bail("cudaGraphAddNode(while)", e);
+    cudaGraph_t body_while = cw.conditional.phGraph_out[0];
+    for (int b = 0; b < 2; ++b) {
+        before = launch_counter();
+        e = cudaStreamBeginCaptureToGraph(stream, b == 0 ? body_if : body_while, nullptr, nullptr, 0, cudaStreamCaptureModeThreadLocal);
+        if (e != cudaSuccess) return bail("cudaStreamBeginCaptureToGraph", e);
+        rc = b == 0 ? record_part(CYCLE_REST) : record_cycle();
+        if (rc == MGB200_OK) { k_loop_check<<<1, 1, 0, stream>>>(h_while, d_norm2, d_loop); rc = check_launch("k_loop_check"); }
+        cudaGraph_t captured = nullptr;
+        e = cudaStreamEndCapture(stream, &captured);
+        (b == 0 ? fold_rest_kernels : loop_kernels) = launch_counter() - before;
+        launch_counter() = before;
+        if (rc != MGB200_OK) return failed(rc);
+        if (e != cudaSuccess) return bail("cudaStreamEndCapture(fold step)", e);
+    }
+    for (size_t l = 0; l < lv.size(); ++l)
+        if (lv[l].cur != cur0[l]) return failed(fail(MGB200_ERR_STATE, "cycle does not restore buffer parity"));
+    e = cudaGraphInstantiate(&fold_exec, graph, 0);
+    if (e != cudaSuccess) { fold_exec = nullptr; return bail("cudaGraphInstantiate(fold step)", e); }
+    cudaGraphDestroy(graph);
+    return MGB200_OK;
+}
+
+int mgb200_solver::fold_step_host(mgb200_solve_info* info)
+{
+    long before = launch_counter();
+    MGB_TRY(record_part(CYCLE_HEAD));
+    count(before);
+    have_rhs = true;
+    double r0 = 0;
+    MGB_TRY(read_norm(&r0));
+    norm_is_res0 = false; res0_on_host = true; res0 = r0;
+    double r = r0;
+    int it = 0;
+    if (info) { std::memset(info, 0, sizeof(*info)); info->hist[0] = r0; }
+    for (; it < opt.max_cycle && r / r0 > tol; ++it) {
+        if (it == 0) {
+            before = launch_counter();
+            MGB_TRY(record_part(CYCLE_REST));
+            count(before);
+            dump_marks();
+        } else {
+            MGB_TRY(run_cycle_async());
+        }
+        MGB_TRY(read_norm(&r));
+        if (info) info->hist[it + 1] = r;
+    }
+    if (it == 0) lv[0].cur = 1 - lv[0].cur;
+    if (info) { info->cycles = it; info->res0 = r0; info->res = r; info->converged = (r / r0 <= tol) ? 1 : 0; }
+    report_solve(it, opt.max_cycle, r0, r, tol);
+    return MGB200_OK;
+}
+
 int mgb200_solver::read_norm(double* out)
 {
     MGB_CUDA(cudaMemcpyAsync(h_norm2, d_norm2, sizeof(double), cudaMemcpyDeviceToHost, stream));
@@ -909,13 +1038,22 @@
 int mgb200_solver::timestep(int nsteps, mgb200_solve_info* infos)
 {
     if (nsteps <= 0) return MGB200_OK;
+    const bool fold = have_fields && folds();
+    if (fold) {
+        if (device_loop() && !fold_exec && build_fold_graph() != MGB200_OK)
+            fprintf(stderr, "mgb200: device-side solve loop unavailable (%s); using the host loop\n", mgb200_last_error());
+        if (!(device_loop() && fold_exec)) {
+            for (int k = 0; k < nsteps; ++k) MGB_TRY(fold_step_host(infos ? &infos[k] : nullptr));
+            return MGB200_OK;
+        }
+    }
     int k0 = 0;
-    if (device_loop() && !loop_exec) {
+    if (!fold && device_loop() && !loop_exec) {
         MGB_TRY(form_rhs(nullptr, false));
         MGB_TRY(solve(infos ? &infos[0] : nullptr));
         k0 = 1;
     }
-    if (!(device_loop() && loop_exec)) {
+    if (!fold && !(device_loop() && loop_exec)) {
         for (int k = k0; k < nsteps; ++k) {
             MGB_TRY(form_rhs(nullptr, false));
             MGB_TRY(solve(infos ? &infos[k] : nullptr));
@@ -931,16 +1069,22 @@
         h_steps_cap = todo;
     }
     for (int k = 0; k < todo; ++k) {
-        MGB_TRY(form_rhs(nullptr, false));
-        MGB_CUDA(cudaGraphLaunch(loop_exec, stream));
+        if (fold) {
+            MGB_CUDA(cudaGraphLaunch(fold_exec, stream));
+        } else {
+            MGB_TRY(form_rhs(nullptr, false));
+            MGB_CUDA(cudaGraphLaunch(loop_exec, stream));
+        }
         MGB_CUDA(cudaMemcpyAsync(&h_steps[k], d_loop, sizeof(LoopState), cudaMemcpyDeviceToHost, stream));
     }
     MGB_CUDA(cudaStreamSynchronize(stream));
+    if (fold) have_rhs = true;
     norm_is_res0 = false; res0_on_host = true;
     for (int k = 0; k < todo; ++k) {
         const LoopState& ls = h_steps[k];
         const int it = ls.iter;
-        launches += 1 + (long)it * loop_kernels;
+        if (fold) launches += fold_head_kernels + (it > 0 ? fold_rest_kernels + (long)(it - 1) * loop_kernels : 0);
+        else launches += 1 + (long)it * loop_kernels;
         res0 = ls.res0; res = ls.hist[it];
         if (infos) {
             mgb200_solve_info& info = infos[k0 + k];
diff --git a/hpcclassmultigridproject_b200/csrc/stream_pass.cuh b/hpcclassmultigridproject_b200/csrc/stream_pass.cuh
--- a/hpcclassmultigridproject_b200/csrc/stream_pass.cuh
+++ b/hpcclassmultigridproject_b200/csrc/stream_pass.cuh
@@ -35,6 +35,7 @@
     long c_own_lo, c_own_hi;
     int* sync;
     int* raise_up; int* raise_dn;
+    double* fold_rhs;
 };
 
 long stream_pass_tiles(long n, long nrows, int iters);
diff --git a/hpcclassmultigridproject_b200/csrc/syst_pass.cu b/hpcclassmultigridproject_b200/csrc/syst_pass.cu
--- a/hpcclassmultigridproject_b200/csrc/syst_pass.cu
+++ b/hpcclassmultigridproject_b200/csrc/syst_pass.cu
@@ -136,7 +136,7 @@
     return x;
 }
 
-template <int ARITH, bool PRE, int POSTK>
+template <int ARITH, bool PRE, int POSTK, bool FOLD = false>
 __global__ void __launch_bounds__(THREADS, 1) k_syst_pass(const __grid_constant__ Params p)
 {
     extern __shared__ __align__(128) unsigned char smem_raw[];
@@ -158,7 +158,7 @@
         if (p.raise_dn && tl.R1 + 8 > (int)p.own_hi) sy_wait_neighbour(p.sync, SYNC_PASS_DOWN);
     }
     __syncthreads();
-    const double acc = run_warp<ARITH, PRE, POSTK>(p, tl, geo, sm, warp, lane);
+    const double acc = run_warp<ARITH, PRE, POSTK, FOLD>(p, tl, geo, sm, warp, lane);
     if (p.sync) {
         const bool pushed = (p.raise_up && tl.rb0 < (int)(p.own_lo + 2 * p.push_rows + 2)) || (p.raise_dn && tl.rb1 > (int)(p.own_hi - 2 * p.push_rows - 2));
         if (pushed) __threadfence_system();
@@ -173,7 +173,7 @@
             }
         }
     }
-    if (POSTK == POST_NORM2) {
+    if (POSTK == POST_NORM2 || FOLD) {
         const double tot = block_sum(acc, scratch);
         if (threadIdx.x == 0) p.partials[blockIdx.x] = tot;
     }
@@ -226,6 +226,16 @@
     return post == POST_NORM2 ? k_syst_pass<ARITH, false, POST_NORM2> : post == POST_INJECT ? k_syst_pass<ARITH, false, POST_INJECT>
                                                                                              : k_syst_pass<ARITH, false, POST_NONE>;
 }
+template <int ARITH>
+static PassKernel fold_kernel_of(int post)
+{
+    return post == POST_FW ? k_syst_pass<ARITH, false, POST_FW, true> : post == POST_INJECT ? k_syst_pass<ARITH, false, POST_INJECT, true>
+                                                                                            : k_syst_pass<ARITH, false, POST_NONE, true>;
+}
+static PassKernel fold_kernel(int arith, int post)
+{
+    return arith == MGB200_ARITH_EXACT ? fold_kernel_of<MGB200_ARITH_EXACT>(post) : fold_kernel_of<MGB200_ARITH_FAST>(post);
+}
 static PassKernel pass_kernel(int arith, bool pre, int post)
 {
     if (post == POST_FW) return arith == MGB200_ARITH_EXACT ? k_syst_pass<MGB200_ARITH_EXACT, false, POST_FW> : k_syst_pass<MGB200_ARITH_FAST, false, POST_FW>;
@@ -249,8 +259,11 @@
         for (int pre = 0; pre < 2; ++pre)
             for (int post = 0; post < 3; ++post)
                 MGB_CUDA(cudaFuncSetAttribute(pass_kernel(arith, pre != 0, post), cudaFuncAttributeMaxDynamicSharedMemorySize, (int)SMEM_BYTES));
-    for (int arith = 0; arith < 2; ++arith)
+    for (int arith = 0; arith < 2; ++arith) {
         MGB_CUDA(cudaFuncSetAttribute(pass_kernel(arith, false, POST_FW), cudaFuncAttributeMaxDynamicSharedMemorySize, (int)SMEM_BYTES));
+        for (int post : {POST_NONE, POST_INJECT, POST_FW})
+            MGB_CUDA(cudaFuncSetAttribute(fold_kernel(arith, post), cudaFuncAttributeMaxDynamicSharedMemorySize, (int)SMEM_BYTES));
+    }
     if (!g_encode) {
         void* fn = nullptr;
         cudaDriverEntryPointQueryResult qres;
@@ -295,7 +308,7 @@
     p.cpitch = a.Lc.pitch; p.codd = a.Lc.odd;
     p.RBAND = pl.RBAND; p.WK = pl.WK; p.SWK = pl.SWK; p.nstrips = pl.nstrips; p.nbands = pl.nbands;
     p.K = a.iters;
-    p.pre = a.coarse_u ? 1 : 0;
+    p.pre = a.coarse_u || a.fold_rhs ? 1 : 0;
     p.post = a.post;
     p.u_is_zero = a.u_in ? 0 : 1;
     p.CW = pl.SWK / 2 + 8;
@@ -307,12 +320,14 @@
     MGB_TRY(encode_field(&p.maps[FIELD_V1], a.v1, a.L.odd, a.L.pitch, p.rows_mem, pl.SWK, GROUP));
     MGB_TRY(encode_field(&p.maps[FIELD_V2], a.v2, a.L.odd, a.L.pitch, p.rows_mem, pl.SWK, GROUP));
     if (a.coarse_u) MGB_TRY(encode_field(&p.maps[FIELD_C], a.coarse_u, a.Lc.odd, a.Lc.pitch, p.crows_mem, p.CW, CROWS));
-    p.u_out = a.u_out; p.crhs = a.coarse_rhs; p.partials = a.partials;
+    p.u_out = a.u_out; p.crhs = a.coarse_rhs; p.partials = a.partials; p.rhs_out = a.fold_rhs;
     p.peer_u_up = a.peer_u_up; p.peer_u_dn = a.peer_u_dn; p.peer_c_up = a.peer_c_up; p.peer_c_dn = a.peer_c_dn;
     p.push_rows = a.push_rows; p.c_own_lo = a.c_own_lo; p.c_own_hi = a.c_own_hi;
     p.sync = a.sync; p.raise_up = a.raise_up; p.raise_dn = a.raise_dn;
     if (p.post == POST_INJECT && !p.crhs) return fail(MGB200_ERR_INVALID, "stream_pass: POST_INJECT without coarse_rhs");
-    if (p.post == POST_FW && (!p.crhs || p.pre)) return fail(MGB200_ERR_INVALID, "stream_pass: POST_FW needs coarse_rhs and no prolongation");
+    if (a.fold_rhs && (a.coarse_u || !a.u_in || !p.partials || p.post == POST_NORM2 || a.push_rows))
+        return fail(MGB200_ERR_INVALID, "stream_pass: a fold pass is a down-leg pass of a single-GPU level with partials");
+    if (p.post == POST_FW && (!p.crhs || a.coarse_u)) return fail(MGB200_ERR_INVALID, "stream_pass: POST_FW needs coarse_rhs and no prolongation");
     if (p.post == POST_NORM2 && !p.partials) return fail(MGB200_ERR_INVALID, "stream_pass: POST_NORM2 without partials");
     grid_out = (unsigned)(pl.nstrips * pl.nbands);
     smem_out = smem_bytes(pl.SWK);
@@ -335,7 +350,7 @@
         key.rows_mem = a.rows_mem; key.crow0 = a.crow0; key.crows_mem = a.crows_mem;
         key.peer_u_up = a.peer_u_up; key.peer_u_dn = a.peer_u_dn; key.peer_c_up = a.peer_c_up; key.peer_c_dn = a.peer_c_dn;
         key.push_rows = a.push_rows; key.c_own_lo = a.c_own_lo; key.c_own_hi = a.c_own_hi; key.sync = a.sync;
-        key.raise_up = a.raise_up; key.raise_dn = a.raise_dn;
+        key.raise_up = a.raise_up; key.raise_dn = a.raise_dn; key.fold_rhs = a.fold_rhs;
         std::string k(reinterpret_cast<const char*>(&key), sizeof(key));
         auto it = cache.find(k);
         if (it == cache.end()) {
@@ -346,7 +361,8 @@
         }
         e = it->second;
     }
-    pass_kernel(a.arith, e.p.pre != 0, e.p.post)<<<e.grid, THREADS, e.smem, s>>>(e.p);
+    if (e.p.rhs_out) fold_kernel(a.arith, e.p.post)<<<e.grid, THREADS, e.smem, s>>>(e.p);
+    else pass_kernel(a.arith, e.p.pre != 0, e.p.post)<<<e.grid, THREADS, e.smem, s>>>(e.p);
     return check_launch("k_syst_pass");
 }
 
diff --git a/hpcclassmultigridproject_b200/csrc/syst_pass_body.cuh b/hpcclassmultigridproject_b200/csrc/syst_pass_body.cuh
--- a/hpcclassmultigridproject_b200/csrc/syst_pass_body.cuh
+++ b/hpcclassmultigridproject_b200/csrc/syst_pass_body.cuh
@@ -57,6 +57,7 @@
     double* peer_u_up; double* peer_u_dn; double* peer_c_up; double* peer_c_dn;
     long push_rows, c_own_lo, c_own_hi;
     int* sync; int* raise_up; int* raise_dn;
+    double* rhs_out;
 };
 
 struct Tile {
@@ -297,6 +298,61 @@
     for (int k = 0; k <= klast; ++k) pre_step(p, tl, geo, sm, st, k);
 }
 
+template <int ARITH, int XR>
+SY_FN void rhs_loop(const Params& p, const Tile& tl, const Geo& geo, const Smem& sm, Stage& st)
+{
+    const int klast = last_step(p, tl, XR) - tl.R0;
+    const unsigned sw = geo.swkb;
+#ifdef SY_HOST_MODEL
+    const bool live = st.live;
+#else
+    const bool live = true;
+#endif
+    const bool wlive = st.live;
+    sy_full_wait(sm, 0, 0u);
+    D2 upE{0.0, 0.0}, upO{0.0, 0.0}, cE{0.0, 0.0}, cO{0.0, 0.0};
+    if (live) { cE = sy_lds2(sm, st.a_cur); cO = sy_lds2(sm, st.a_cur + sw); }
+    for (int k = 0; k <= klast; ++k) {
+        const int t = st.row;
+        if (((k + 1) & (GROUP - 1)) == 0 && t + 1 <= tl.R1) {
+            const int g = (k + 1) / GROUP;
+            sy_full_wait(sm, g % NGROUP, (unsigned)(g / NGROUP) & 1u);
+        }
+        D2 dnE{0.0, 0.0}, dnO{0.0, 0.0};
+        if (t + 1 <= tl.R1 && live) { dnE = sy_lds2(sm, st.a_next); dnO = sy_lds2(sm, st.a_next + sw); }
+        if (t > tl.R0 && t < tl.R1) {
+            D2 aE{0.0, 0.0}, aO{0.0, 0.0}, bE{0.0, 0.0}, bO{0.0, 0.0};
+            if (live) {
+                aE = sy_lds2(sm, st.a_cur + 2u * geo.ringb); aO = sy_lds2(sm, st.a_cur + 2u * geo.ringb + sw);
+                bE = sy_lds2(sm, st.a_cur + 3u * geo.ringb); bO = sy_lds2(sm, st.a_cur + 3u * geo.ringb + sw);
+            }
+            const double lfE = sy_side(sm, cO, st.a_cur + sw - 8u, -1, st.outer_l);
+            const double rtO = sy_side(sm, cE, st.a_cur + 16u, 1, st.outer_r);
+            const Coef4 kE0 = Arith<ARITH>::coef(aE.x, bE.x, p.st), kE1 = Arith<ARITH>::coef(aE.y, bE.y, p.st);
+            const Coef4 kO0 = Arith<ARITH>::coef(aO.x, bO.x, p.st), kO1 = Arith<ARITH>::coef(aO.y, bO.y, p.st);
+            const double fE0 = Arith<ARITH>::rhs(cE.x, upE.x, lfE, dnE.x, cO.x, kE0, p.st);
+            const double fE1 = Arith<ARITH>::rhs(cE.y, upE.y, cO.x, dnE.y, cO.y, kE1, p.st);
+            const double fO0 = Arith<ARITH>::rhs(cO.x, upO.x, cE.x, dnO.x, cE.y, kO0, p.st);
+            const double fO1 = Arith<ARITH>::rhs(cO.y, upO.y, cE.y, dnO.y, rtO, kO1, p.st);
+            const bool row_int = t >= 1 && t <= (int)p.n - 1;
+            const unsigned mE = row_int ? st.cmask0 : 0u, mO = row_int ? st.cmask1 : 0u;
+            if (wlive) {
+                sy_sts2(sm, st.a_cur + geo.ringb, D2{(mE & 1u) ? fE0 : 0.0, (mE & 2u) ? fE1 : 0.0});
+                sy_sts2(sm, st.a_cur + geo.ringb + sw, D2{(mO & 1u) ? fO0 : 0.0, (mO & 2u) ? fO1 : 0.0});
+            }
+            if (t >= st.elo && t <= st.ehi) {
+                if (st.rmask0 & 1u) { const double r = Arith<ARITH>::residual(fE0, cE.x, upE.x, lfE, dnE.x, cO.x, kE0, p.st); st.acc += r * r; }
+                if (st.rmask1 & 1u) { const double r = Arith<ARITH>::residual(fO0, cO.x, upO.x, cE.x, dnO.x, cE.y, kO0, p.st); st.acc += r * r; }
+                if (st.rmask0 & 2u) { const double r = Arith<ARITH>::residual(fE1, cE.y, upE.y, cO.x, dnE.y, cO.y, kE1, p.st); st.acc += r * r; }
+                if (st.rmask1 & 2u) { const double r = Arith<ARITH>::residual(fO1, cO.y, upO.y, cE.y, dnO.y, rtO, kO1, p.st); st.acc += r * r; }
+            }
+        }
+        publish(sm, st, k);
+        upE = cE; upO = cO; cE = dnE; cO = dnO;
+        advance_row(geo, st);
+    }
+}
+
 SY_FN void store_coarse(const Params& p, const Stage& st, long kg, long cr, double r0, double r1)
 {
     double* crow = p.crhs + (cr - p.crow0) * p.cpitch + (kg >> 1);
@@ -454,30 +510,31 @@
         stage_step<ARITH, LAST, NORM1, RESID, EPI, false>(p, tl, geo, sm, st, k, par, true, &fw);
 }
 
+template <bool FOLD = false>
 SY_FN void issue_group_loads(const Params& p, const Tile& tl, const Geo& geo, const Smem& sm, int g)
 {
     if (!sy_elect()) return;
     const int gs = g % NGROUP;
     const int z = tl.R0 + GROUP * g - (int)p.row0;
     const unsigned fine = (unsigned)GROUP * geo.rowb;
-    sy_full_expect(sm, gs, 4u * fine + (p.pre ? geo.cgrpb : 0u));
+    sy_full_expect(sm, gs, FOLD ? 3u * fine : 4u * fine + (p.pre ? geo.cgrpb : 0u));
     const unsigned so = (unsigned)gs * fine;
     sy_tma_load(p, sm, FIELD_U, so, tl.k0, p.u_is_zero ? (int)p.rows_mem + 64 : z, gs);
-    sy_tma_load(p, sm, FIELD_F, so + geo.ringb, tl.k0, z, gs);
+    if (!FOLD) sy_tma_load(p, sm, FIELD_F, so + geo.ringb, tl.k0, z, gs);
     sy_tma_load(p, sm, FIELD_V1, so + 2u * geo.ringb, tl.k0, z, gs);
     sy_tma_load(p, sm, FIELD_V2, so + 3u * geo.ringb, tl.k0, z, gs);
-    if (p.pre)
+    if (!FOLD && p.pre)
         sy_tma_load(p, sm, FIELD_C, 4u * geo.ringb + (unsigned)gs * geo.cgrpb, tl.k0 / 2, ((z + (int)p.row0) >> 1) - (int)p.crow0, gs);
     const int zp = z + 2 * GROUP;
     if (g + 2 >= NGROUP && zp + (int)p.row0 <= tl.R1) {
         if (!p.u_is_zero) sy_tma_prefetch(p, FIELD_U, tl.k0, zp);
-        sy_tma_prefetch(p, FIELD_F, tl.k0, zp);
+        if (!FOLD) sy_tma_prefetch(p, FIELD_F, tl.k0, zp);
         sy_tma_prefetch(p, FIELD_V1, tl.k0, zp);
         sy_tma_prefetch(p, FIELD_V2, tl.k0, zp);
     }
 }
 
-template <int XR = 0>
+template <int XR = 0, bool FOLD = false>
 SY_FN void store_loop(const Params& p, const Tile& tl, const Geo& geo, const Smem& sm)
 {
     const int klast = last_step(p, tl, XR) - tl.R0;
@@ -510,6 +567,11 @@
                 sy_fence_async();
                 if (nE8) sy_bulk_store(sm, gstE, a, nE8);
                 if (nO8) sy_bulk_store(sm, gstO, a + geo.swkb, nO8);
+                if (FOLD && rs >= 1 && rs <= (int)p.n - 1) {
+                    double* fE = p.rhs_out + ((long)rs - p.row0) * pitch + tl.kb;
+                    if (nE8) sy_bulk_store(sm, fE, a + geo.ringb, nE8);
+                    if (nO8) sy_bulk_store(sm, fE + p.odd, a + geo.ringb + geo.swkb, nO8);
+                }
                 if (push) {
                     if (p.peer_u_up && rs < p.own_lo + p.push_rows) {
                         double* q = p.peer_u_up + (long)rs * pitch + tl.kb;
@@ -536,12 +598,12 @@
     if (sy_elect()) { sy_store_commit(); sy_store_wait_all(); sy_prog_publish(sm, 2 * PAIR_STORE, groups + 64u); }
 }
 
-template <int XR = 0>
+template <int XR = 0, bool FOLD = false>
 SY_FN void producer_loop(const Params& p, const Tile& tl, const Geo& geo, const Smem& sm)
 {
     const int ng = num_groups(tl);
     int gnext = 0;
-    for (; gnext < ng && gnext < NGROUP; ++gnext) issue_group_loads(p, tl, geo, sm, gnext);
+    for (; gnext < ng && gnext < NGROUP; ++gnext) issue_group_loads<FOLD>(p, tl, geo, sm, gnext);
     const int klast = last_step(p, tl, XR) - tl.R0;
     const int pair_s = 2 * p.K - 1, off_s = off_stage(p, pair_s);
     const bool epi = p.post != POST_NONE;
@@ -553,12 +615,12 @@
         prog_wait(sm, pair_l, (unsigned)k + 1u, need_h1 * ((unsigned)k + 1u), sy_prog_peek(sm, pair_l));
         prog_wait(sm, PAIR_STORE, (unsigned)(gnext - NGROUP + 1), 0u, sy_prog_peek(sm, PAIR_STORE));
         if (sy_elect()) sy_fence_async();
-        issue_group_loads(p, tl, geo, sm, gnext);
+        issue_group_loads<FOLD>(p, tl, geo, sm, gnext);
         ++gnext;
     }
 }
 
-template <int ARITH, bool PRE, int POSTK>
+template <int ARITH, bool PRE, int POSTK, bool FOLD = false>
 SY_FN double run_warp(const Params& p, const Tile& tl, const Geo& geo, const Smem& sm, int warp, int lane)
 {
     constexpr int XR = POSTK == POST_FW ? 2 : 0;
@@ -566,20 +628,25 @@
 #ifdef SY_HOST_MODEL
         if (lane != 0) return 0.0;
 #endif
-        producer_loop<XR>(p, tl, geo, sm);
+        producer_loop<XR, FOLD>(p, tl, geo, sm);
         return 0.0;
     }
     if (warp == STORE_WARP) {
 #ifdef SY_HOST_MODEL
         if (lane != 0) return 0.0;
 #endif
-        store_loop<XR>(p, tl, geo, sm);
+        store_loop<XR, FOLD>(p, tl, geo, sm);
         return 0.0;
     }
     const int pair = warp / NSTW, h = warp % NSTW;
     if (h >= geo.nh) return 0.0;
     const int last = 2 * p.K - 1;
     if (pair == PAIR_PRE) {
+        if (FOLD) {
+            Stage st = init_role(p, tl, geo, PAIR_PRE, -1, 0, 0, h, lane);
+            rhs_loop<ARITH, XR>(p, tl, geo, sm, st);
+            return st.acc;
+        }
         if (!PRE) return 0.0;
         Stage st = init_role(p, tl, geo, PAIR_PRE, -1, 1, 0, h, lane);
         pre_loop(p, tl, geo, sm, st);
@@ -592,7 +659,7 @@
         return st.acc;
     }
     if (pair > last) return 0.0;
-    Stage st = init_role(p, tl, geo, pair, pair == 0 ? (PRE ? PAIR_PRE : -1) : pair - 1, pair, off_stage(p, pair), h, lane);
+    Stage st = init_role(p, tl, geo, pair, pair == 0 ? (PRE || FOLD ? PAIR_PRE : -1) : pair - 1, pair, off_stage(p, pair), h, lane);
     if (pair == last && POSTK == POST_NORM2) stage_loop<ARITH, true, true, false, POST_NONE>(p, tl, geo, sm, st);
     else if (pair == last && POSTK == POST_FW) stage_loop<ARITH, true, false, false, POST_FW, XR>(p, tl, geo, sm, st);
     else stage_loop<ARITH, false, false, false, POST_NONE, XR>(p, tl, geo, sm, st);
```

New measurement: 6.472, median of 6. -2.2%, faster.
